# manuelruder/fast-artistic-videos

Hardware: AMD Instinct MI355X
Metric: stylized frames/sec @1280x720, per-frame hot path (mask + warp + assembly + net + deprocess + PNG encode on the GPU) with inputs resident in HBM; file->PNG rate of the product CLI (BASELINE.json's end-to-end) in `end_to_end_fps` / `e2e`, PSNR vs CPU ref in `parity` (higher is better)
Workload: dtype f32

## Files before the change

fast-artistic-videos_amd/csrc/fav_internal.h:

```cpp
#pragma once
#include <hip/hip_runtime.h>
#include <cstdarg>
#include <cstdint>
#include <cstdio>
#include <exception>
#include <new>
#include <string>
#include <vector>

#include "../../include/fav.h"

#include <cstdlib>
inline const char* diag_env(const char* name)
{
#ifdef FAV_DIAG
    return getenv(name);
#else
    (void)name;
    return nullptr;
#endif
}

namespace fav {

void set_error(const char* fmt, ...);
int hip_fail(hipError_t e, const char* what);

#define FAV_HIP(expr)                                              \
    do {                                                           \
        hipError_t e__ = (expr);                                   \
        if (e__ != hipSuccess) return ::fav::hip_fail(e__, #expr); \
    } while (0)
#define FAV_LAUNCH_CHECK(name)                                            \
    do {                                                                  \
        hipError_t e__ = hipGetLastError();                               \
        if (e__ != hipSuccess) return ::fav::hip_fail(e__, "launch " name); \
    } while (0)
#define FAV_REQUIRE(cond, ...)                 \
    do {                                       \
        if (!(cond)) {                         \
            ::fav::set_error(__VA_ARGS__);     \
            return FAV_EINVAL;                 \
        }                                      \
    } while (0)

#define FAV_ABI_TRY try {
#define FAV_ABI_CATCH(where_)                                                                                            \
    } catch (const std::bad_alloc&) {                                                                                   \
        ::fav::set_error(where_ ": out of memory while parsing (damaged size field?)"); return FAV_EFORMAT;                \
    } catch (const std::exception& e__) {                                                                               \
        ::fav::set_error(where_ ": %s", e__.what()); return FAV_EFORMAT;                                                  \
    } catch (...) {                                                                                                     \
        ::fav::set_error(where_ ": unexpected exception"); return FAV_EFORMAT;                                            \
    }

int ensure_device();

struct TraceRange {
    explicit TraceRange(const char* name);
    ~TraceRange();
    static bool enabled();
    bool on;
};

enum LayerType { L_PAD, L_CONV, L_IN, L_RELU, L_RES, L_UP, L_TANH, L_MUL, L_IDENTITY, L_BN };

struct Layer {
    LayerType type = L_IDENTITY;
    int pl = 0, pr = 0, pt = 0, pb = 0, pad_mode = 0;
    int cin = 0, cout = 0, k = 0, stride = 1, pad = 0;
    int transposed = 0, adj = 0;
    std::vector<float> w, b;
    std::vector<float> gamma, beta, mean, var;
    float eps = 1e-5f;
    int scale = 1;
    float mul = 1.f;
    int shave = 0;
    std::vector<Layer> block;
};

int t7_parse_model(const char* path, std::vector<Layer>& out);
int blob_pack(const std::vector<Layer>& layers, std::vector<uint8_t>& blob);
int blob_unpack(const void* blob, size_t bytes, std::vector<Layer>& out);
std::string describe_layers(const std::vector<Layer>& layers, int indent = 0);

struct Affine {
    const float* scale1 = nullptr; const float* shift1 = nullptr; int relu1 = 0;
    const float* scale2 = nullptr; const float* shift2 = nullptr; int relu2 = 0;
    int stages = 0;
    const long long* acc1 = nullptr; long long* acc1_zero = nullptr;
    const float* gamma1 = nullptr; const float* beta1 = nullptr; float eps1 = 0.f; int count1 = 0;
};
constexpr int STAT_COPIES = 8;
inline size_t stat_acc_words(int C) { return (size_t)STAT_COPIES * C * 4; }
constexpr long long STAT_NONFINITE = 1ll << 53;
__host__ __device__ inline bool stat_acc_poisoned(long long hi_sum, long long hi_squares)
{
    return hi_sum >= STAT_NONFINITE / 2 || hi_sum <= -(STAT_NONFINITE / 2) || hi_squares >= STAT_NONFINITE / 2 || hi_squares <= -(STAT_NONFINITE / 2);
}

struct ConvLaunch {
    const float* in = nullptr;
    int IH = 0, IW = 0;
    int IWp = 0;
    int ups = 0;
    int stuff = 0;
    int CIN = 0;
    Affine pre;
    const float* wgt = nullptr;
    const unsigned short* wgt16 = nullptr;
    const float* bias = nullptr;
    int COUT = 0, COUTp = 0;
    int KH = 0, KW = 0, stride = 1, pad = 0;
    int Kpad = 0;
    int OH = 0, OW = 0;
    float* out = nullptr;
    float* partials = nullptr;
    int final_mode = 0;
    float tanh_mul = 1.f;
    float* out_planar = nullptr;
    float* out_raw_nchw = nullptr;
    float* sk_ws = nullptr; unsigned* sk_flags = nullptr; unsigned sk_epoch = 0;
    unsigned* sk_err = nullptr;
    int reserve_cus = 0;
    int no_sk = 0;
    const float* join_skip = nullptr; float* join_out = nullptr; int OWp = 0;
    long long* stat_acc = nullptr;
    float* ks_ws = nullptr; int* ks_cnt = nullptr;
};
inline size_t conv3_wino4_ksplit_bytes() { return (size_t)256 * 2 * 256 * 128 * sizeof(float); }
size_t conv_streamk_workspace_bytes();
int conv_streamk_grid();
constexpr int CONV_BM = 128;
inline int conv_mblocks(int OH, int OW) { return (OH * OW + CONV_BM - 1) / CONV_BM; }
int launch_conv(const ConvLaunch& p, hipStream_t st);
bool conv_c8_eligible(int cin_pitch, int coutp, int k, int stride, int stages, int ups);
int conv_c8_tiles(int OH, int OW);
int launch_conv_c8(const ConvLaunch& p, int* counts, hipStream_t st);
bool conv_c8d_eligible(int cin_pitch, int cin_real, int coutp, int k, int stride, int stages, int ups);
void conv_c8d_pack(const float* w, int cin, int cout, std::vector<float>& out);
int launch_conv_c8d(const ConvLaunch& p, int cin_real, const float* wc8d, int* counts, hipStream_t st);
bool conv3_halo_eligible(int cin_pitch, int coutp, int k, int stride);
int conv3_halo_tiles(int OH, int OW, bool edge_b);
int launch_conv3_halo(const ConvLaunch& p, int* counts, hipStream_t st);
bool conv3s2_eligible(int cin_pitch, int coutp, int k, int stride, int stages, int ups);
int conv3s2_tiles(int OH, int OW);
int launch_conv3s2(const ConvLaunch& p, int* counts, hipStream_t st);
bool conv_fold_eligible(int cin_pitch, int cout, int k, int stride);
bool conv_fold_launchable(int cin_pitch, int k, int pad, int ups, int IH, int IW);
int launch_conv_fold(const ConvLaunch& p, const float* wfold, hipStream_t st);
int conv_first_tiles(int OH, int OW);
int launch_conv_first(const ConvLaunch& p, int cin_real, const float* wpk, int* counts, hipStream_t st);
bool conv_first2d_eligible(int cin_pitch, int cin_real, int coutp, int k, int stride, int stages, int ups);
int conv_first2d_tiles(int OH, int OW);
int launch_conv_first2d(const ConvLaunch& p, int cin_real, const float* wpk, int* counts, hipStream_t st);
bool conv3_wino_eligible(int cin_pitch, int cout, int coutp, int k, int stride, int pad, int stages, int ups);
int conv3_wino_tiles(int OH, int OW);
int launch_conv3_wino(const ConvLaunch& p, const float* wpk, int* counts, hipStream_t st);
bool conv3_wino4_eligible(int cin_pitch, int cout, int coutp, int k, int stride, int pad, int stages, int ups);
int conv3_wino4_tiles(int OH, int OW);
int launch_conv3_wino4(const ConvLaunch& p, const float* wpk, int* counts, hipStream_t st);
bool conv3_up2_eligible(int cin_pitch, int cout, int coutp, int k, int stride, int pad, int stages, int ups);
int conv3_up2_tiles(int OH, int OW);
int launch_conv3_up2(const ConvLaunch& p, const float* wpk, int* counts, hipStream_t st);
bool conv3s2w_eligible(int cin_pitch, int cout, int coutp, int k, int stride, int pad, int stages, int ups);
int conv3s2w_tiles(int OH, int OW, int coutp);
int launch_conv3s2w(const ConvLaunch& p, const float* wpk, int* counts, hipStream_t st);
enum ConvKernel { CK_GENERIC, CK_FOLD, CK_C8, CK_C8D, CK_FIRST1D, CK_FIRST2D, CK_S2W, CK_UP2, CK_WINO, CK_WINO4, CK_HALO3, CK_S2HALO };
constexpr int CONV_KERNELS = CK_S2HALO + 1;
int launch_in_finalize(const float* partials, const int* counts, int mblocks, int M, int block_pixels, int C, int Cpitch,
                       const float* gamma, const float* beta, float eps,
                       float* scale, float* shift, hipStream_t st);
int launch_stats(const float* x, int M, int C, const Affine& t, float* partials, hipStream_t st);
int launch_pad_nhwc(const float* in, int Hp, int Wp, int in_pitch, int C, int ups, float* out, int pl, int pr, int pt, int pb, int mode, hipStream_t st);
int launch_res_add(const float* y, const float* scale, const float* shift,
                   const float* skip, int SH, int SW, int shave, const Affine& skip_t,
                   int C, float* z, float* partials, int* counts, hipStream_t st, int skip_pitch = 0, const Affine* branch_acc = nullptr);
inline int res_add_stat_blocks(int OH, int OW) { return OH * ((OW + 127) / 128); }
int launch_nchw_to_nhwc_pad(const float* in, int C, int H, int W, int pad, int Cp, float* out, hipStream_t st);
int launch_nhwc_to_nchw(const float* in, int M, int C, const Affine& t, float* out, hipStream_t st);

#ifdef __HIPCC__
__device__ __forceinline__ float fill_uniform(unsigned seed, unsigned index, unsigned c, unsigned y, unsigned x)
{
    unsigned k = seed * 0x9E3779B1u + index * 0x85EBCA77u + c * 0xC2B2AE3Du + y * 0x27D4EB2Fu + x * 0x165667B1u;
    k ^= k >> 15; k *= 0x2C1B3C6Du;
    k ^= k >> 12; k *= 0x297A2D39u;
    k ^= k >> 15;
    return (float)(k >> 8) * (1.0f / 16777216.0f);
}
#endif

int launch_warp(const float* img, const float* flow, float* out, int B, int C, int H, int W, int Ho, int Wo,
                int border, hipStream_t st);
int launch_min_filter_f32(const float* cert, float* out, int H, int W, int r, hipStream_t st);
int launch_assemble(const float* frame, const float* warped, const float* cert, float* in7, int H, int W,
                    hipStream_t st);
int launch_cert_prepare(const uint8_t* mask, const float* backward_flo, int invert, int fix_occ, int border,
                        int r, float* cert_tmp, float* cert, int H, int W, hipStream_t st);
int launch_prep_input(const uint8_t* frame_hwc, const float* prev_rgb, int Hs, int Ws, const float* backward_flo,
                      const float* cert, int border, int H, int W, int pad, float* in8, hipStream_t st,
                      int fill_random = 0, unsigned seed = 0, unsigned index = 0, int* q0_out = nullptr);
int launch_quantize_rgb8(const float* rgb_planar, uint8_t* out_hwc, int H, int W, hipStream_t st);
int launch_scale_prep(const uint8_t* frame_hwc, int H, int W, int Hs, int Ws, int pad, float* in8, hipStream_t st,
                      int fill_random = 0, unsigned seed = 0, unsigned index = 0);
int launch_scale_planar(const float* src, float* dst, int C, int Hs, int Ws, int Hd, int Wd, hipStream_t st);
constexpr int PNG_NSYM = 277;
constexpr int PNG_NTABLES = 12;
constexpr int PNG_HDR_WORDS = 40;
struct PngTable {
    uint32_t sym[PNG_NSYM];
    uint32_t hdr[PNG_HDR_WORDS];
    uint32_t hdr_bits, btype, dist_len, dist_code;
};
const std::vector<PngTable>& png_tables();
size_t png_capacity(int W, int H);
size_t png_workspace_bytes(int W, int H);
uint32_t png_crc32_combine_host(uint32_t crc_a, uint32_t crc_b, uint32_t len_b);
int launch_png_encode(const uint8_t* rgb_hwc, const float* rgb_planar, int W, int H, void* png_out, size_t capacity, uint32_t* png_bytes,
                      void* workspace, size_t ws_bytes, hipStream_t st);
int launch_check_cert(const float* backward_flo, const float* forward_flo, const float* structure, const float* avg, uint8_t* mask_out,
                      int invert, int fix_occ, int border, int r, float* cert, int H, int W, hipStream_t st);
int launch_check_prep(const uint8_t* frame_hwc, const float* prev_rgb, int Hs, int Ws, const float* backward_flo, const float* forward_flo,
                      const float* structure, const float* avg, uint8_t* mask_out, float* cert, int invert, int fix_occ, int border, int r,
                      int H, int W, int pad, float* in8, hipStream_t st, int fill_random, unsigned seed, unsigned index);
int launch_store_flag(uint32_t* flag_host, uint32_t value, hipStream_t st);
int launch_unpad_input(const float* in8, int H, int W, int pad, float* in7, hipStream_t st);
int launch_temporal_loss(const float* prev_rgb, const float* cur_rgb, const float* backward_flo, const uint8_t* cert_u8, int border,
                         int H, int W, double* partial256, hipStream_t st);

size_t structure_workspace_bytes(int W, int H);
int launch_structure(const uint8_t* rgb_hwc, int W, int H, void* ws, size_t ws_bytes,
                     const float** structure_out, const float** avg_out, hipStream_t st, int pack_cus = 0, const int* q0_main = nullptr);
int launch_sequential_sum(const float* x, size_t n, float* sum_out, hipStream_t st);
int launch_consistency(const float* f1_flo, const float* f2_flo, const float* structure, const float* avg,
                       uint8_t* out, int W, int H, hipStream_t st);

int launch_vr_rotate(const float* src, float* dst, int H, int W, int mode, hipStream_t st);
int launch_vr_accum(float* acc, const float* w, const float* div, size_t n, int first, hipStream_t st);
int launch_vr_cert(const uint8_t* cert_u8, const float* m0, const float* m1, const float* m2, const float* m3, float* out, size_t n,
                   hipStream_t st);
int launch_vr_prior(const float* lfw, const float* border, const float* grad, const float* cert, const float* m, const float* m2,
                    float* out, size_t n, hipStream_t st);
int launch_vr_blend(const float* seg, const float* borders, const float* g, const float* anti, float* out, size_t n, hipStream_t st);
int launch_vr_median(const float* src, float* dst, int H, int W, int r, hipStream_t st);
int launch_vr_strip(const float* face, int FH, int FW, int cy, int cx, int CH, int CW, int mode, float* strip, int SH, int SW,
                    int x0, hipStream_t st);
int launch_vr_prep(const uint8_t* frame_hwc, const float* prior, const float* cert, int fill_random, unsigned seed, unsigned index,
                   int H, int W, int pad, float* in8, hipStream_t st);
int launch_vr_flo_to_lua(const float* flo_uv, float* lua_dydx, size_t n, hipStream_t st);

}

struct fav_net;
namespace fav {
int net_device(const fav_net* n);
int net_pad(const fav_net* n);
int net_in_channels(const fav_net* n);
void net_out_size(const fav_net* n, int H, int W, int* Ho, int* Wo);
int net_forward_padded(fav_net* n, const float* in8, int H, int W, float* out_planar, hipStream_t st);
void net_forget_stream(const fav_net* n, hipStream_t st);
void net_reserve_cus(fav_net* n, int cus);
}
```

fast-artistic-videos_amd/csrc/kernels_elem.hip:

```cpp
#include <algorithm>

#include "fav_internal.h"
#include "conv_device.h"

namespace fav {

namespace {

__global__ __launch_bounds__(256) void in_finalize_kernel(const float2* partials, const int* counts, int mblocks, int M, int bp,
                                                          int Cpitch, const float* gamma, const float* beta,
                                                          float eps, float* scale, float* shift)
{
    __shared__ double sh[8];
    const int c = blockIdx.x, t = threadIdx.x;
    double s1 = 0, s2 = 0;
    float gq = 1.f, bq = 0.f;
    if (t == 0) { gq = gamma ? gamma[c] : 1.f; bq = beta ? beta[c] : 0.f; }
    for (int b0 = t; b0 < mblocks; b0 += 1024) {
        float2 pr[4]; int nb[4];
#pragma unroll
        for (int k = 0; k < 4; ++k) {
            const int b = b0 + 256 * k, bc = min(b, mblocks - 1);
            pr[k] = partials[(size_t)bc * Cpitch + c];
            nb[k] = b < mblocks ? (counts ? counts[bc] : min(bp, M - bc * bp)) : 0;
        }
#pragma unroll
        for (int k = 0; k < 4; ++k) {
            const double n = (double)nb[k], mu = (double)pr[k].x;
            s1 += n * mu;
            s2 += (nb[k] ? (double)pr[k].y : 0.0) + n * mu * mu;
        }
    }
    for (int o = 32; o > 0; o >>= 1) { s1 += __shfl_xor(s1, o); s2 += __shfl_xor(s2, o); }
    if ((t & 63) == 0) { sh[2 * (t >> 6)] = s1; sh[2 * (t >> 6) + 1] = s2; }
    __syncthreads();
    if (t == 0) {
        const double a = ((sh[0] + sh[2]) + sh[4]) + sh[6], q = ((sh[1] + sh[3]) + sh[5]) + sh[7];
        const double mean = a / (double)M;
        double var = q / (double)M - mean * mean;
        var = var > 0.0 ? var : 0.0;
        const double g = (double)gq, bt = (double)bq;
        const double sc = g / sqrt(var + (double)eps);
        scale[c] = (float)sc;
        shift[c] = (float)(bt - mean * sc);
    }
}

__device__ __forceinline__ float4 apply_affine_g(float4 v, const Affine& a, int c)
{
    if (a.stages >= 1) {
        v = affine4(v, a.scale1 + c, a.shift1 + c, a.relu1);
        if (a.stages >= 2) v = affine4(v, a.scale2 + c, a.shift2 + c, a.relu2);
    }
    return v;
}

template <int NPT>
__global__ __launch_bounds__(256) void stats_kernel(const float* x, int M, int C, const Affine a, float2* partials)
{
    __shared__ float red[1024];
    __shared__ float mean_s[1024];
    const int t = threadIdx.x;
    const int groups = C >> 2;
    const int nl = 256 / groups;
    const int g = t % groups, pl = t / groups;
    const int m0 = blockIdx.x * 128;
    const int cnt = min(128, M - m0);
    const bool active = pl < nl;
    float4 s = make_float4(0, 0, 0, 0);
    float4 keep[NPT > 0 ? NPT : 1];
    if (NPT > 0) {
#pragma unroll
        for (int i = 0; i < NPT; ++i) {
            const int pix = pl + i * nl;
            float4 v = make_float4(0, 0, 0, 0);
            if (pix < cnt) { v = *reinterpret_cast<const float4*>(x + (size_t)(m0 + pix) * C + 4 * g); v = apply_affine_g(v, a, 4 * g); }
            keep[i] = v;
        }
#pragma unroll
        for (int i = 0; i < NPT; ++i) { s.x += keep[i].x; s.y += keep[i].y; s.z += keep[i].z; s.w += keep[i].w; }
    } else if (active)
        for (int pix = pl; pix < cnt; pix += nl) {
            float4 v = *reinterpret_cast<const float4*>(x + (size_t)(m0 + pix) * C + 4 * g);
            v = apply_affine_g(v, a, 4 * g);
            s.x += v.x; s.y += v.y; s.z += v.z; s.w += v.w;
        }
    if (active) *reinterpret_cast<float4*>(red + pl * C + 4 * g) = s;
    __syncthreads();
    for (int c = t; c < C; c += 256) {
        float r = 0;
        for (int i = 0; i < nl; ++i) r += red[i * C + c];
        mean_s[c] = r / (float)cnt;
    }
    __syncthreads();
    float4 q = make_float4(0, 0, 0, 0);
    if (active) {
        const float4 mu = *reinterpret_cast<const float4*>(mean_s + 4 * g);
        if (NPT > 0) {
#pragma unroll
            for (int i = 0; i < NPT; ++i) {
                const float4 v = keep[i];
                const float dx = v.x - mu.x, dy = v.y - mu.y, dz = v.z - mu.z, dw = v.w - mu.w;
                if (pl + i * nl < cnt) { q.x = fmaf(dx, dx, q.x); q.y = fmaf(dy, dy, q.y); q.z = fmaf(dz, dz, q.z); q.w = fmaf(dw, dw, q.w); }
            }
        } else
            for (int pix = pl; pix < cnt; pix += nl) {
                float4 v = *reinterpret_cast<const float4*>(x + (size_t)(m0 + pix) * C + 4 * g);
                v = apply_affine_g(v, a, 4 * g);
                const float dx = v.x - mu.x, dy = v.y - mu.y, dz = v.z - mu.z, dw = v.w - mu.w;
                q.x = fmaf(dx, dx, q.x); q.y = fmaf(dy, dy, q.y); q.z = fmaf(dz, dz, q.z); q.w = fmaf(dw, dw, q.w);
            }
        *reinterpret_cast<float4*>(red + pl * C + 4 * g) = q;
    }
    __syncthreads();
    for (int c = t; c < C; c += 256) {
        float r = 0;
        for (int i = 0; i < nl; ++i) r += red[i * C + c];
        partials[(size_t)blockIdx.x * C + c] = make_float2(mean_s[c], r);
    }
}

template <bool ACC>
__global__ __launch_bounds__(256) void res_add_kernel(const float* y, const float* scale, const float* shift,
                                                      const float* skip, int SW, int shave, const Affine sa,
                                                      int OH, int OW, int C, float* z, const Affine br)
{
    __shared__ float ss[ACC ? 2048 : 4];
    if (ACC) {
        for (int i = threadIdx.x; i < C; i += 256) {
            long long w0 = 0, w1 = 0, w2 = 0, w3 = 0;
#pragma unroll
            for (int cp = 0; cp < STAT_COPIES; ++cp) {
                const longlong2* a = reinterpret_cast<const longlong2*>(br.acc1 + ((size_t)cp * C + i) * 4);
                const longlong2 lo = a[0], hi = a[1];
                w0 += lo.x; w1 += lo.y; w2 += hi.x; w3 += hi.y;
            }
            const double s1 = ((double)w1 * 4294967296.0 + (double)w0) * (1.0 / 1099511627776.0);
            const double s2 = ((double)w3 * 4294967296.0 + (double)w2) * (1.0 / 1099511627776.0);
            const double mean = s1 / (double)br.count1;
            double var = s2 / (double)br.count1 - mean * mean;
            var = var > 0.0 ? var : 0.0;
            const double sc = stat_acc_poisoned(w1, w3) ? (double)NAN : (double)br.gamma1[i] / sqrt(var + (double)br.eps1);
            ss[i] = (float)sc; ss[C + i] = (float)((double)br.beta1[i] - mean * sc);
            if (blockIdx.x == 0) {
#pragma unroll
                for (int cp = 0; cp < STAT_COPIES; ++cp) {
                    longlong2* zz = reinterpret_cast<longlong2*>(br.acc1_zero + ((size_t)cp * C + i) * 4);
                    zz[0] = longlong2{0, 0}; zz[1] = longlong2{0, 0};
                }
            }
        }
        __syncthreads();
        scale = ss; shift = ss + C;
    }
    const int groups = C >> 2;
    const size_t total = (size_t)OH * OW * groups;
    for (size_t idx = (size_t)blockIdx.x * 256 + threadIdx.x; idx < total; idx += (size_t)gridDim.x * 256) {
        const int g = (int)(idx % groups);
        const size_t pix = idx / groups;
        const int oy = (int)(pix / OW), ox = (int)(pix - (size_t)oy * OW);
        float4 v = *reinterpret_cast<const float4*>(y + pix * C + 4 * g);
        v = affine4(v, scale + 4 * g, shift + 4 * g, 0);
        float4 k = *reinterpret_cast<const float4*>(skip + ((size_t)(oy + shave) * SW + ox + shave) * C + 4 * g);
        k = apply_affine_g(k, sa, 4 * g);
        v.x += k.x; v.y += k.y; v.z += k.z; v.w += k.w;
        *reinterpret_cast<float4*>(z + pix * C + 4 * g) = v;
    }
}

template <int NPT>
__global__ __launch_bounds__(256) void res_add_stats_kernel(const float* y, const float* scale, const float* shift,
                                                            const float* skip, int SW, int shave, const Affine sa,
                                                            int OW, int C, float* z, float2* partials, int* counts)
{
    __shared__ float red[1024];
    __shared__ float mean_s[1024];
    const int t = threadIdx.x;
    const int groups = C >> 2, nl = 256 / groups;
    const int g = t % groups, pl = t / groups;
    const int segs = (OW + 127) / 128;
    const int oy = blockIdx.x / segs, x0 = (blockIdx.x - oy * segs) * 128;
    const int cnt = min(128, OW - x0);
    const bool active = pl < nl;
    const float* yr = y + ((size_t)oy * OW + x0) * C + 4 * g;
    const float* kr = skip + ((size_t)(oy + shave) * SW + x0 + shave) * C + 4 * g;
    float* zr = z + ((size_t)oy * OW + x0) * C + 4 * g;
    float4 sm = make_float4(0, 0, 0, 0);
    float4 keep[NPT > 0 ? NPT : 1];
    if (NPT > 0) {
        float4 kk[NPT > 0 ? NPT : 1];
#pragma unroll
        for (int i = 0; i < NPT; ++i) {
            const int px = pl + i * nl;
            keep[i] = make_float4(0, 0, 0, 0); kk[i] = make_float4(0, 0, 0, 0);
            if (px < cnt) { keep[i] = *reinterpret_cast<const float4*>(yr + (size_t)px * C); kk[i] = *reinterpret_cast<const float4*>(kr + (size_t)px * C); }
        }
#pragma unroll
        for (int i = 0; i < NPT; ++i) {
            const int px = pl + i * nl;
            float4 v = affine4(keep[i], scale + 4 * g, shift + 4 * g, 0);
            const float4 k = apply_affine_g(kk[i], sa, 4 * g);
            v.x += k.x; v.y += k.y; v.z += k.z; v.w += k.w;
            if (px < cnt) { *reinterpret_cast<float4*>(zr + (size_t)px * C) = v; sm.x += v.x; sm.y += v.y; sm.z += v.z; sm.w += v.w; }
            keep[i] = v;
        }
    } else if (active)
        for (int px = pl; px < cnt; px += nl) {
            float4 v = *reinterpret_cast<const float4*>(yr + (size_t)px * C);
            v = affine4(v, scale + 4 * g, shift + 4 * g, 0);
            float4 k = *reinterpret_cast<const float4*>(kr + (size_t)px * C);
            k = apply_affine_g(k, sa, 4 * g);
            v.x += k.x; v.y += k.y; v.z += k.z; v.w += k.w;
            *reinterpret_cast<float4*>(zr + (size_t)px * C) = v;
            sm.x += v.x; sm.y += v.y; sm.z += v.z; sm.w += v.w;
        }
    if (active) *reinterpret_cast<float4*>(red + pl * C + 4 * g) = sm;
    __syncthreads();
    for (int c = t; c < C; c += 256) {
        float r = 0;
        for (int i = 0; i < nl; ++i) r += red[i * C + c];
        mean_s[c] = r / (float)cnt;
    }
    __syncthreads();
    float4 q = make_float4(0, 0, 0, 0);
    if (active) {
        const float4 mu = *reinterpret_cast<const float4*>(mean_s + 4 * g);
        if (NPT > 0) {
#pragma unroll
            for (int i = 0; i < NPT; ++i) {
                const float4 v = keep[i];
                const float dx = v.x - mu.x, dy = v.y - mu.y, dz = v.z - mu.z, dw = v.w - mu.w;
                if (pl + i * nl < cnt) { q.x = fmaf(dx, dx, q.x); q.y = fmaf(dy, dy, q.y); q.z = fmaf(dz, dz, q.z); q.w = fmaf(dw, dw, q.w); }
            }
        } else
        for (int px = pl; px < cnt; px += nl) {
            const float4 v = *reinterpret_cast<const float4*>(zr + (size_t)px * C);
            const float dx = v.x - mu.x, dy = v.y - mu.y, dz = v.z - mu.z, dw = v.w - mu.w;
            q.x = fmaf(dx, dx, q.x); q.y = fmaf(dy, dy, q.y); q.z = fmaf(dz, dz, q.z); q.w = fmaf(dw, dw, q.w);
        }
        *reinterpret_cast<float4*>(red + pl * C + 4 * g) = q;
    }
    __syncthreads();
    for (int c = t; c < C; c += 256) {
        float r = 0;
        for (int i = 0; i < nl; ++i) r += red[i * C + c];
        partials[(size_t)blockIdx.x * C + c] = make_float2(mean_s[c], r);
    }
    if (t == 0) counts[blockIdx.x] = cnt;
}

__device__ __forceinline__ int reflect(int i, int n)
{
    if (i < 0) i = -i;
    if (i >= n) i = 2 * (n - 1) - i;
    return i;
}

__global__ __launch_bounds__(256) void nchw_to_nhwc_pad_kernel(const float* in, int C, int H, int W, int pad, int Cp,
                                                               float* out)
{
    const int Hp = H + 2 * pad, Wp = W + 2 * pad;
    const size_t total = (size_t)Hp * Wp * Cp;
    for (size_t idx = (size_t)blockIdx.x * 256 + threadIdx.x; idx < total; idx += (size_t)gridDim.x * 256) {
        const int c = (int)(idx % Cp);
        const size_t pix = idx / Cp;
        const int y = (int)(pix / Wp), x = (int)(pix - (size_t)y * Wp);
        float v = 0.f;
        if (c < C) v = in[((size_t)c * H + reflect(y - pad, H)) * W + reflect(x - pad, W)];
        out[idx] = v;
    }
}

__global__ __launch_bounds__(256) void nhwc_to_nchw_kernel(const float* in, int M, int C, const Affine a, float* out)
{
    const size_t total = (size_t)M * C;
    for (size_t idx = (size_t)blockIdx.x * 256 + threadIdx.x; idx < total; idx += (size_t)gridDim.x * 256) {
        const int c = (int)(idx / M);
        const size_t m = idx - (size_t)c * M;
        float v = in[m * C + c];
        if (a.stages >= 1) {
            v = fmaf(v, a.scale1[c], a.shift1[c]); if (a.relu1) v = fmaxf(v, 0.f);
            if (a.stages >= 2) { v = fmaf(v, a.scale2[c], a.shift2[c]); if (a.relu2) v = fmaxf(v, 0.f); }
        }
        out[idx] = v;
    }
}

inline int grid_for(size_t total) { size_t b = (total + 255) / 256; return (int)(b > 8192 ? 8192 : (b ? b : 1)); }

}

int launch_in_finalize(const float* partials, const int* counts, int mblocks, int M, int block_pixels, int C, int Cpitch,
                       const float* gamma, const float* beta, float eps, float* scale, float* shift, hipStream_t st)
{
    hipLaunchKernelGGL(in_finalize_kernel, dim3(C), dim3(256), 0, st, reinterpret_cast<const float2*>(partials), counts,
                       mblocks, M, block_pixels, Cpitch, gamma, beta, eps, scale, shift);
    FAV_LAUNCH_CHECK("in_finalize_kernel");
    return FAV_OK;
}

int launch_stats(const float* x, int M, int C, const Affine& t, float* partials, hipStream_t st)
{
    FAV_REQUIRE(C % 4 == 0 && C <= 1024 && 256 % (C / 4) == 0, "stats: unsupported channel count %d", C);
    const dim3 grid((M + 127) / 128);
    float2* pp = reinterpret_cast<float2*>(partials);
    if (C == 64) hipLaunchKernelGGL(stats_kernel<8>, grid, dim3(256), 0, st, x, M, C, t, pp);
    else if (C == 128) hipLaunchKernelGGL(stats_kernel<16>, grid, dim3(256), 0, st, x, M, C, t, pp);
    else hipLaunchKernelGGL(stats_kernel<0>, grid, dim3(256), 0, st, x, M, C, t, pp);
    FAV_LAUNCH_CHECK("stats_kernel");
    return FAV_OK;
}

int launch_res_add(const float* y, const float* scale, const float* shift, const float* skip, int SH, int SW,
                   int shave, const Affine& skip_t, int C, float* z, float* partials, int* counts, hipStream_t st, int skip_pitch, const Affine* branch_acc)
{
    const int OH = SH - 2 * shave, OW = SW - 2 * shave;
    if (skip_pitch > 0) SW = skip_pitch;
    FAV_REQUIRE(C % 4 == 0 && C <= 1024 && 256 % (C / 4) == 0 && OH > 0 && OW > 0, "res_add: bad shape (C=%d)", C);
    FAV_REQUIRE(!(partials && branch_acc && branch_acc->acc1), "res_add: the statistics-taking join does not take an accumulator-form InstanceNorm");
    if (partials) {
        const dim3 grid(res_add_stat_blocks(OH, OW));
        float2* pp = reinterpret_cast<float2*>(partials);
        if (C == 128) hipLaunchKernelGGL(res_add_stats_kernel<16>, grid, dim3(256), 0, st, y, scale, shift, skip, SW, shave, skip_t, OW, C, z, pp, counts);
        else if (C == 64) hipLaunchKernelGGL(res_add_stats_kernel<8>, grid, dim3(256), 0, st, y, scale, shift, skip, SW, shave, skip_t, OW, C, z, pp, counts);
        else hipLaunchKernelGGL(res_add_stats_kernel<0>, grid, dim3(256), 0, st, y, scale, shift, skip, SW, shave, skip_t, OW, C, z, pp, counts);
    }
    else if (branch_acc != nullptr && branch_acc->acc1 != nullptr)
        hipLaunchKernelGGL(res_add_kernel<true>, dim3(std::min(1024, grid_for((size_t)OH * OW * (C / 4)))), dim3(256), 0, st, y, scale, shift, skip, SW, shave, skip_t,
                           OH, OW, C, z, *branch_acc);
    else
        hipLaunchKernelGGL(res_add_kernel<false>, dim3(grid_for((size_t)OH * OW * (C / 4))), dim3(256), 0, st, y, scale, shift, skip, SW, shave, skip_t,
                           OH, OW, C, z, Affine());
    FAV_LAUNCH_CHECK("res_add_kernel");
    return FAV_OK;
}

int launch_nchw_to_nhwc_pad(const float* in, int C, int H, int W, int pad, int Cp, float* out, hipStream_t st)
{
    FAV_REQUIRE(pad < H && pad < W, "reflection pad %d must be smaller than the image (%dx%d)", pad, W, H);
    hipLaunchKernelGGL(nchw_to_nhwc_pad_kernel, dim3(grid_for((size_t)(H + 2 * pad) * (W + 2 * pad) * Cp)), dim3(256), 0,
                       st, in, C, H, W, pad, Cp, out);
    FAV_LAUNCH_CHECK("nchw_to_nhwc_pad_kernel");
    return FAV_OK;
}

int launch_nhwc_to_nchw(const float* in, int M, int C, const Affine& t, float* out, hipStream_t st)
{
    hipLaunchKernelGGL(nhwc_to_nchw_kernel, dim3(grid_for((size_t)M * C)), dim3(256), 0, st, in, M, C, t, out);
    FAV_LAUNCH_CHECK("nhwc_to_nchw_kernel");
    return FAV_OK;
}

}
```

fast-artistic-videos_amd/csrc/kernels_wino4.hip:

```cpp
#include <algorithm>
#include <cstdlib>
#include <type_traits>
#include <vector>

#include "fav_internal.h"
#include "wino4_pack.h"

namespace fav {

typedef float v4f __attribute__((ext_vector_type(4)));
typedef int v4i __attribute__((ext_vector_type(4)));

namespace {

constexpr int MAX_DEVICES = 64;
constexpr int W4_MEET_MAX = 256;
constexpr int W4_SHARES = 252;
inline int cur_dev() { int d = 0; (void)hipGetDevice(&d); return (d >= 0 && d < MAX_DEVICES) ? d : 0; }

constexpr int W4_VPOS = 256;
constexpr int W4_VBUF = 36 * W4_VPOS;
constexpr int W4_LLINE = 18 * 4;
constexpr int W4_LTY = 113 * 4;
constexpr int W4_LKQ = 464 * 4;
constexpr int W4_LBUF = 4 * W4_LKQ;
constexpr int W4_RBUF = 6 * 288 * 4;
constexpr int W4_SMEM = 2 * W4_VBUF + W4_LBUF + W4_RBUF;
static_assert((W4_LTY / 4) % 16 == 1 && (W4_LKQ / 4) % 16 == 0 && W4_LTY >= 6 * W4_LLINE && W4_LKQ >= 4 * W4_LTY, "pitches of L");

struct Wino4Args {
    const float* in; const float* wpk; const float* bias; const float* scale1; const float* shift1;
    float* out; float2* partials; int* counts;
    const float* skip; float* zout;
    int OWp;
    int IH, IW, IWp, CIN, OH, OW, units_x, units_y, relu1;
    int stream, shares; float* ks_ws; int* ks_cnt;
    long long* dbg;
    long long* stat_acc; const long long* acc1; long long* acc1_zero; const float* gamma1; const float* beta1; float eps1; int count1;
    int COUT, groups;
};

__device__ __forceinline__ void w4_store16_wt(void* ptr, v4f v)
{
    asm volatile("global_store_dwordx4 %0, %1, off sc1" ::"v"(ptr), "v"(v) : "memory");
}

typedef float v2f __attribute__((ext_vector_type(2)));
__device__ __forceinline__ v2f w4_fma(float a, v2f b, v2f c) { return __builtin_elementwise_fma(v2f{a, a}, b, c); }
__device__ __forceinline__ void w4_bt2(const v2f d[6], v2f v[6])
{
    const v2f e1 = w4_fma(-2.25f, d[2], d[4]), o1 = w4_fma(-1.6875f, d[1], 0.75f * d[3]);
    const v2f e2 = w4_fma(-0.5625f, d[2], d[4]), o2 = w4_fma(-0.84375f, d[1], 1.5f * d[3]);
    v[0] = w4_fma(1.265625f, d[0], w4_fma(-2.8125f, d[2], d[4]));
    v[1] = e1 + o1; v[2] = e1 - o1; v[3] = e2 + o2; v[4] = e2 - o2;
    v[5] = w4_fma(1.265625f, d[1], w4_fma(-2.8125f, d[3], d[5]));
}
__device__ __forceinline__ void w4_bt(const v4f d[6], v4f v[6])
{
    v2f dl[6], dh[6], vl[6], vh[6];
#pragma unroll
    for (int i = 0; i < 6; ++i) { dl[i] = d[i].xy; dh[i] = d[i].zw; }
    w4_bt2(dl, vl); w4_bt2(dh, vh);
#pragma unroll
    for (int i = 0; i < 6; ++i) v[i] = v4f{vl[i].x, vl[i].y, vh[i].x, vh[i].y};
}
__device__ __forceinline__ void w4_at(const v2f m[6], v2f y[4])
{
    const v2f s1 = m[1] + m[2], d1 = m[1] - m[2], s2 = m[3] + m[4], d2 = m[3] - m[4];
    y[0] = (m[0] + s1) + s2;
    y[1] = w4_fma(1.5f, d2, 0.75f * d1);
    y[2] = w4_fma(2.25f, s2, 0.5625f * s1);
    y[3] = w4_fma(3.375f, d2, w4_fma(0.421875f, d1, m[5]));
}

template <int MODE, int VAR = 0, bool WIDE = false>
__global__ __launch_bounds__(512) __attribute__((amdgpu_waves_per_eu(2, 2))) void conv3_wino4_kernel(const Wino4Args p)
{
    constexpr bool AFF = MODE != 0, JOIN = MODE == 2;
    constexpr bool PAIR = (VAR & 8) == 0 && MODE != 2;
    constexpr int NT = 512;
    extern __shared__ __attribute__((aligned(16))) float smem[];
    float* const Vs = smem;
    float* const Ls = smem + 2 * W4_VBUF;
    float* const Rs = Ls + W4_LBUF;
    float* const Ss = Rs + W4_RBUF;
    float* const aff = Ss + ((MODE == 2 || PAIR) ? W4_RBUF : 0);
    typedef __attribute__((address_space(3))) void* lds_ptr_t;

    const int t = threadIdx.x, lane = t & 63;
    const int wave = __builtin_amdgcn_readfirstlane(t >> 6);
    const int CIN = p.CIN, nslices = CIN >> 4;

    int dbi = 0;
#define DBG_T() { if (p.dbg && t == 0 && dbi < 21) p.dbg[blockIdx.x * 24 + dbi++] = wall_clock64(); }
    DBG_T();
    int lb;
    {
        const int nwg = gridDim.x, q = nwg >> 3, r = nwg & 7, xcd = blockIdx.x & 7, idx = blockIdx.x >> 3;
        lb = (xcd < r ? xcd * (q + 1) : r * (q + 1) + (xcd - r) * q) + idx;
    }
    if (MODE == 1 && p.acc1 != nullptr) {
        for (int i = t; i < CIN; i += NT) {
            long long w0 = 0, w1 = 0, w2 = 0, w3 = 0;
#pragma unroll
            for (int cp = 0; cp < STAT_COPIES; ++cp) {
                const longlong2* a = reinterpret_cast<const longlong2*>(p.acc1 + ((size_t)cp * CIN + i) * 4);
                const longlong2 lo = a[0], hi = a[1];
                w0 += lo.x; w1 += lo.y; w2 += hi.x; w3 += hi.y;
            }
            const double s1 = ((double)w1 * 4294967296.0 + (double)w0) * (1.0 / 1099511627776.0);
            const double s2 = ((double)w3 * 4294967296.0 + (double)w2) * (1.0 / 1099511627776.0);
            const double mean = s1 / (double)p.count1;
            double var = s2 / (double)p.count1 - mean * mean;
            var = var > 0.0 ? var : 0.0;
            const double sc = stat_acc_poisoned(w1, w3) ? (double)NAN : (double)p.gamma1[i] / sqrt(var + (double)p.eps1);
            aff[i] = (float)sc; aff[CIN + i] = (float)((double)p.beta1[i] - mean * sc);
            if (blockIdx.x == 0) {
#pragma unroll
                for (int cp = 0; cp < STAT_COPIES; ++cp) {
                    longlong2* z = reinterpret_cast<longlong2*>(p.acc1_zero + ((size_t)cp * CIN + i) * 4);
                    z[0] = longlong2{0, 0}; z[1] = longlong2{0, 0};
                }
            }
        }
    } else if (AFF) for (int i = t; i < CIN; i += NT) { aff[i] = p.scale1[i]; aff[CIN + i] = p.shift1[i]; }
    const float lo1 = (MODE == 1 && p.relu1) ? 0.f : -INFINITY;

    const bool has1 = t < 288;
    const int cq = (t >> 3) & 3;
    const int pix1 = min((t >> 5) * 8 + (t & 7), 71), ty1 = (pix1 * 3641) >> 16, x1 = pix1 - ty1 * 18;
    float* const l1 = Ls + cq * W4_LKQ + ty1 * W4_LTY + x1 * 4;
    const float* const affr = aff + cq * 4;
    const bool has2 = wave >= 2;
    const int i2 = max(wave - 2, 0);
    const int m2 = lane & 15, kq2 = lane >> 4;
    const float* const l2 = Ls + kq2 * W4_LKQ + (m2 >> 2) * W4_LTY + 4 * (m2 & 3) * 4 + i2 * W4_LLINE;
    float* const v2 = Vs + lane * 4 + 6 * i2 * W4_VPOS;
    const float* const aA = Vs + lane * 4;
    const int wlo = lane * 16, wso = wave * 1024;

    v4f fb[6];
    bool ring_primed = false;
    int ring_grp = 0;
    const int upix = p.units_x * p.units_y;
    if (AFF) __syncthreads();
    auto work = [&](const int ug, const int s0, const int s1, const int meet, const int part) {
        const int nsl = s1 - s0;
        const bool whole = meet < 0;
        if (s0 != 0) ring_primed = false;
        int u = ug, grp = 0;
        if (WIDE) {
            if (p.stream) { grp = ug / upix; u = ug - grp * upix; } else { u = ug / p.groups; grp = ug - u * p.groups; }
            if (grp != ring_grp) { ring_primed = false; ring_grp = grp; }
        }
        const int wgb = (p.CIN >> 4) * 36 * 8192;
        const __amdgpu_buffer_rsrc_t wrs = __builtin_amdgcn_make_buffer_rsrc(const_cast<float*>(p.wpk) + (WIDE ? (size_t)grp * (wgb >> 2) : 0), 0, wgb, 0x00020000);
        const __amdgpu_buffer_rsrc_t irs = __builtin_amdgcn_make_buffer_rsrc(const_cast<float*>(p.in), 0, p.IH * p.IWp * p.CIN * 4, 0x00020000);
        const __amdgpu_buffer_rsrc_t srs = __builtin_amdgcn_make_buffer_rsrc(const_cast<float*>(JOIN ? p.skip : p.in), 0, p.IH * p.IWp * p.CIN * 4, 0x00020000);
        const __amdgpu_buffer_rsrc_t zrs = __builtin_amdgcn_make_buffer_rsrc(JOIN ? p.zout : const_cast<float*>(p.in), 0, p.IH * p.IWp * p.CIN * 4, 0x00020000);
        const int uy = u / p.units_x, ux = u - uy * p.units_x;
        const int oy0 = uy * 16, ox0 = ux * 16;
        DBG_T();
        const int ho0 = ((min(oy0 + 4 * ty1, p.IH - 1) * p.IWp + min(ox0 + x1, p.IW - 1)) * CIN + cq * 4) * 4;
        const int hrmax = max(p.IH - 1 - (oy0 + 4 * ty1), 0);
        const int hrow = p.IWp * CIN * 4;
#define ho_(a_) (ho0 + min((a_), hrmax) * hrow)
        const int dpix = min(t >> 2, 71), dty = (dpix * 3641) >> 16, dx = dpix - dty * 18;
        const int hd0 = ((min(oy0 + 4 * dty, p.IH - 1) * p.IWp + min(ox0 + dx, p.IW - 1)) * CIN + (t & 3) * 4) * 4;
        const int hdmax = max(p.IH - 1 - (oy0 + 4 * dty), 0);
#define hd_(a_) (hd0 + min((a_), hdmax) * hrow)
        int zm = 0;
        const bool lastx = ux == p.units_x - 1, lasty = uy == p.units_y - 1;
        if (JOIN) {
            const bool cv = ox0 + x1 < p.IW && (x1 < 16 || lastx);
#pragma unroll
            for (int a = 0; a < 6; ++a) zm |= (cv && oy0 + 4 * ty1 + a < p.IH && (a < 4 || (ty1 == 3 && lasty)) ? 1 : 0) << a;
        }

        v4f sc, sh;
        float* const land = Rs + wave * 256;
        const float* const rread = Rs + (pix1 * 4 + cq) * 4;
        constexpr int RROW = 288 * 4;
        constexpr int SKO = W4_RBUF;
#define W4_LOAD_RAW(q_, slice_)                                                                     \
        { _Pragma("unroll") for (int a = 0; a < 6; ++a) q_[a] = __builtin_bit_cast(v4f, __builtin_amdgcn_raw_buffer_load_b128(irs, ho_(a), (slice_) * 64, 0)); }
#define W4_LOAD_SKIP(x_, slice_)                                                                    \
        { if (JOIN) { _Pragma("unroll") for (int a = 0; a < 6; ++a) x_[a] = __builtin_bit_cast(v4f, __builtin_amdgcn_raw_buffer_load_b128(srs, ho_(a), (slice_) * 64, 0)); } }
#define W4_REQ_RAW(slice_)                                                                          \
        { asm volatile("" ::: "memory");       \
          if (JOIN) { _Pragma("unroll") for (int a = 0; a < 6; ++a)      \
              __builtin_amdgcn_raw_ptr_buffer_load_lds(srs, (lds_ptr_t)(land + SKO + a * RROW), 16, hd_(a), (slice_) * 64, 0, 0); } \
          _Pragma("unroll") for (int a = 0; a < 6; ++a)                                             \
              __builtin_amdgcn_raw_ptr_buffer_load_lds(irs, (lds_ptr_t)(land + a * RROW), 16, hd_(a), (slice_) * 64, 0, 0); }
#define W4_TAKE_RAW(q_)                                                                             \
        { _Pragma("unroll") for (int a = 0; a < 6; ++a) q_[a] = *reinterpret_cast<const v4f*>(rread + a * RROW); }
        constexpr int RROW2 = 576 * 4;
        const float* const rread2 = Rs + (pix1 * 8 + cq) * 4;
        float* const land2 = Rs + wave * 512;
#define W4_REQ_PAIR(a_)                                                                             \
        { asm volatile("" ::: "memory");                                                            \
          int ln_ = lane; asm volatile("" : "+v"(ln_));                                             \
          _Pragma("unroll") for (int j = 0; j < 2; ++j) { if (j == 0 || wave < 4) {                 \
              const int dp_ = 16 * wave + 8 * j + (ln_ >> 3), dy_ = (dp_ * 3641) >> 16, dx_ = dp_ - 18 * dy_;                     \
              const int b_ = ((min(oy0 + 4 * dy_, p.IH - 1) * p.IWp + min(ox0 + dx_, p.IW - 1)) * CIN + (ln_ & 7) * 4) * 4;       \
              const int mx_ = max(p.IH - 1 - (oy0 + 4 * dy_), 0);                                   \
              _Pragma("unroll") for (int a = 0; a < 6; ++a)                                         \
                  __builtin_amdgcn_raw_ptr_buffer_load_lds(irs, (lds_ptr_t)(land2 + j * 256 + a * RROW2), 16, b_ + min(a, mx_) * hrow, (a_) * 64, 0, 0); } } }
#define W4_TAKE_PAIR(q_, slice_)                                                                    \
        { const float* const rr_ = rread2 + ((slice_) & 1) * 16;                                     \
          _Pragma("unroll") for (int a = 0; a < 6; ++a) q_[a] = *reinterpret_cast<const v4f*>(rr_ + a * RROW2); }
#define W4_SKIP_LDS(a_) (*reinterpret_cast<const v4f*>(rread + SKO + (a_) * RROW))
#define W4_AFF(slice_)                                                                              \
        { if (AFF) { sc = *reinterpret_cast<const v4f*>(affr + (slice_) * 16); sh = *reinterpret_cast<const v4f*>(affr + CIN + (slice_) * 16); } }
#define W4_PEND(q_, xs_, slice_)                                                                    \
        { _Pragma("unroll") for (int a = 0; a < 6; ++a) {                                           \
            if (MODE == 1) { const v2f fl_ = __builtin_elementwise_fma(q_[a].xy, sc.xy, sh.xy), fh_ = __builtin_elementwise_fma(q_[a].zw, sc.zw, sh.zw); \
                             q_[a].x = fmaxf(fl_.x, lo1); q_[a].y = fmaxf(fl_.y, lo1); q_[a].z = fmaxf(fh_.x, lo1); q_[a].w = fmaxf(fh_.y, lo1); } \
            if (JOIN) { const v4f x1_ = xs_(a);                                                     \
                        q_[a].x = fmaf(q_[a].x, sc.x, sh.x) + x1_.x; q_[a].y = fmaf(q_[a].y, sc.y, sh.y) + x1_.y;                \
                        q_[a].z = fmaf(q_[a].z, sc.z, sh.z) + x1_.z; q_[a].w = fmaf(q_[a].w, sc.w, sh.w) + x1_.w;                \
                        if (!(VAR & 16) && (a < 4 || lasty)) __builtin_amdgcn_raw_buffer_store_b128(__builtin_bit_cast(v4i, q_[a]), zrs, (zm & (1 << a)) ? ho_(a) : (int)0xFFFFFFF0, (slice_) * 64, 0); } } }
#define W4_COMMIT1(q_)                                                                              \
        { v4f l_[6]; w4_bt(q_, l_);                                                                 \
          _Pragma("unroll") for (int i = 0; i < 6; ++i) *reinterpret_cast<v4f*>(l1 + i * W4_LLINE) = l_[i]; }
#define W4_S2_READ(c_)                                                                              \
        { _Pragma("unroll") for (int k = 0; k < 6; ++k) c_[k] = *reinterpret_cast<const v4f*>(l2 + k * 4); }
#define W4_S2_DONE(c_, nb_)                                                                         \
        { v4f o_[6]; w4_bt(c_, o_);                                                                 \
          _Pragma("unroll") for (int j = 0; j < 6; ++j) *reinterpret_cast<v4f*>(v2 + (nb_) * W4_VBUF + j * W4_VPOS) = o_[j]; }

        v4f fa[4];
#define W4_READ_A(slot_, par_, pos_) { fa[slot_] = *reinterpret_cast<const v4f*>(aA + (par_) * W4_VBUF + (pos_) * W4_VPOS); }
#define W4_LOAD_B(slot_, sl_, pos_)                                                                 \
        { fb[slot_] = __builtin_bit_cast(v4f, __builtin_amdgcn_raw_buffer_load_b128(wrs, wlo, wso + ((sl_) * 36 + (pos_)) * 8192, 0)); }

        {
            v4f qa[6], xa[6];
            if (has1) { W4_LOAD_SKIP(xa, s0); W4_LOAD_RAW(qa, s0); }
            if (!ring_primed) {
#pragma unroll
                for (int q = 0; q < 4; ++q) { W4_LOAD_B(q, s0, q); }
                ring_primed = true;
            }
            if (has1) {
                W4_AFF(s0);
#define W4_SKIP_REG(a_) xa[a_]
                W4_PEND(qa, W4_SKIP_REG, s0); W4_COMMIT1(qa);
#undef W4_SKIP_REG
                if (!PAIR) W4_REQ_RAW(min(s0 + 1, s1 - 1));
            }
            if (PAIR && wave < 5) W4_REQ_PAIR((s0 + 1) & ~1);
            __syncthreads();
            if (has2) { v4f c2[6]; W4_S2_READ(c2); W4_S2_DONE(c2, 0); }
        }
        v4f acc[36];
#pragma unroll
        for (int q = 0; q < 36; ++q) acc[q] = v4f{0.f, 0.f, 0.f, 0.f};
        __syncthreads();
        W4_READ_A(0, 0, 0); W4_READ_A(1, 0, 1);
        DBG_T();
        const long long ck0 = p.dbg ? clock64() : 0, wk0 = p.dbg ? wall_clock64() : 0;

#define W4_FENCE() __builtin_amdgcn_sched_barrier(0)
#define W4_POSITIONS(from_, to_)                                                                    \
        { _Pragma("unroll") for (int pos = (from_); pos < (to_); pos += 2) {                       \
            if (pos + 2 < 36) { W4_READ_A((pos + 2) % 4, par, pos + 2); W4_READ_A((pos + 3) % 4, par, pos + 3); }    \
            if (!(VAR & 1)) {                                                                       \
            if (pos + 4 < 36) { W4_LOAD_B((pos + 4) % 6, s, pos + 4); } else { W4_LOAD_B((pos + 4) % 6, sw, pos + 4 - 36); } \
            if (pos + 5 < 36) { W4_LOAD_B((pos + 5) % 6, s, pos + 5); } else { W4_LOAD_B((pos + 5) % 6, sw, pos + 5 - 36); } } \
            W4_FENCE();                                                                             \
            _Pragma("unroll") for (int j = 0; j < 4; ++j) {                                         \
                acc[pos] = __builtin_amdgcn_mfma_f32_16x16x4f32(fa[pos % 4][j], fb[pos % 6][j], acc[pos], 0, 0, 0); \
                acc[pos + 1] = __builtin_amdgcn_mfma_f32_16x16x4f32(fa[(pos + 1) % 4][j], fb[(pos + 1) % 6][j], acc[pos + 1], 0, 0, 0); \
            }                                                                                       \
            W4_FENCE(); } }
        for (int sl = 0; sl < nsl; ++sl) {
            const int s = s0 + sl, par = sl & 1;
            const int sn = min(s + 1, s1 - 1);
            const int sw = s + 1 < s1 ? s + 1 : 0;
            const int sn2 = min(s + 2, s1 - 1);
            W4_POSITIONS(0, 6);
            if (sl == 0) {
                if (PAIR ? wave < 5 : has1) asm volatile("s_waitcnt vmcnt(6)" ::: "memory");
                __syncthreads();
            }
            if (PAIR) {
                if (has1) { v4f qa[6]; W4_TAKE_PAIR(qa, sn); W4_AFF(sn); W4_PEND(qa, W4_SKIP_LDS, sn); W4_COMMIT1(qa); }
                if (wave < 5 && !(s & 1) && s + 2 < s1) W4_REQ_PAIR(s + 2);
            } else
            if (!(VAR & 2) && has1) {
                v4f qa[6];
                W4_TAKE_RAW(qa);
                W4_AFF(sn); W4_PEND(qa, W4_SKIP_LDS, sn); W4_COMMIT1(qa);
                W4_REQ_RAW(sn2);
            }
            W4_POSITIONS(6, 12);
            if (!(VAR & 4)) __syncthreads();
            W4_POSITIONS(12, 14);
            if (!(VAR & 2) && has2) { v4f c2[6]; W4_S2_READ(c2); W4_S2_DONE(c2, par ^ 1); }
            W4_POSITIONS(14, 36);
            if (PAIR ? wave < 5 : has1) asm volatile("s_waitcnt vmcnt(6)" ::: "memory");
            if (!(VAR & 4)) __syncthreads();
            W4_READ_A(0, par ^ 1, 0); W4_READ_A(1, par ^ 1, 1);
        }
#undef W4_POSITIONS
#undef W4_FENCE
        DBG_T();
        if (p.dbg && t == 0) { p.dbg[blockIdx.x * 24 + 21] += clock64() - ck0; p.dbg[blockIdx.x * 24 + 22] += wall_clock64() - wk0; }
        DBG_T();
#undef ho_
#undef hd_
#undef W4_LOAD_RAW
#undef W4_REQ_RAW
#undef W4_TAKE_RAW
#undef W4_REQ_PAIR
#undef W4_TAKE_PAIR
#undef W4_SKIP_LDS
#undef W4_S2_READ
#undef W4_S2_DONE
#undef W4_LOAD_SKIP
#undef W4_AFF
#undef W4_PEND
#undef W4_COMMIT1
#undef W4_READ_A
#undef W4_LOAD_B

        const int cn = lane & 15, g = lane >> 4;
        const int nrows = max(0, min(16, p.OH - oy0)), ncols = max(0, min(16, p.OW - ox0));
        const int nv = nrows * ncols;
        const int cpb = WIDE ? p.COUT * 4 : 512;
        const __amdgpu_buffer_rsrc_t ors = __builtin_amdgcn_make_buffer_rsrc(p.out, 0, p.OH * p.OWp * cpb, 0x00020000);
        const bool inside = nv == 256;
        const int oyb = oy0 + 4 * g;
        const int cb = (WIDE ? grp * 128 : 0) + wave * 16 + cn;
        float y[4][4][4];
        {
            const float bv = whole ? p.bias[cb] : 0.f;
            const v2f bv2 = v2f{bv, bv};
#pragma unroll
            for (int r = 0; r < 4; r += 2) {
                v2f Q[4][6];
#pragma unroll
                for (int j = 0; j < 6; ++j) {
                    const v2f mcol[6] = {r ? acc[j].zw : acc[j].xy, r ? acc[6 + j].zw : acc[6 + j].xy, r ? acc[12 + j].zw : acc[12 + j].xy,
                                         r ? acc[18 + j].zw : acc[18 + j].xy, r ? acc[24 + j].zw : acc[24 + j].xy, r ? acc[30 + j].zw : acc[30 + j].xy};
                    v2f o[4]; w4_at(mcol, o);
                    Q[0][j] = o[0]; Q[1][j] = o[1]; Q[2][j] = o[2]; Q[3][j] = o[3];
                }
#pragma unroll
                for (int a = 0; a < 4; ++a) {
                    v2f o[4]; w4_at(Q[a], o);
#pragma unroll
                    for (int b = 0; b < 4; ++b) { const v2f ob = o[b] + bv2; y[a][b][r] = ob.x; y[a][b][r + 1] = ob.y; }
                }
            }
        }
        if (!whole) {
            float* const mine = p.ks_ws + ((size_t)meet * 2 + part) * 32768 + (wave * 64 + lane) * 4;
            const float* const other = p.ks_ws + ((size_t)meet * 2 + (part ^ 1)) * 32768 + (wave * 64 + lane) * 4;
            int* const flag = reinterpret_cast<int*>(aff + 2 * CIN);
            if (t == 0) *flag = __hip_atomic_load(p.ks_cnt + meet, __ATOMIC_RELAXED, __HIP_MEMORY_SCOPE_AGENT);
            __syncthreads();
            bool second = *flag == 1;
            __syncthreads();
            if (!second) {
#pragma unroll
                for (int a = 0; a < 4; ++a)
#pragma unroll
                    for (int b = 0; b < 4; ++b)
                        w4_store16_wt(mine + (a * 4 + b) * 2048, v4f{y[a][b][0], y[a][b][1], y[a][b][2], y[a][b][3]});
                asm volatile("s_waitcnt vmcnt(0)" ::: "memory");
                __syncthreads();
                if (t == 0) *flag = __hip_atomic_fetch_add(p.ks_cnt + meet, 1, __ATOMIC_RELAXED, __HIP_MEMORY_SCOPE_AGENT);
                __syncthreads();
                second = *flag == 1;
                __syncthreads();
                if (!second) { DBG_T(); return; }
            }
            __builtin_amdgcn_fence(__ATOMIC_ACQUIRE, "agent");
            if (t == 0) __hip_atomic_store(p.ks_cnt + meet, 0, __ATOMIC_RELAXED, __HIP_MEMORY_SCOPE_AGENT);
            const float bv = p.bias[cb];
#pragma unroll
            for (int a = 0; a < 4; ++a)
#pragma unroll
                for (int b = 0; b < 4; ++b) {
                    const v4f o = *reinterpret_cast<const v4f*>(other + (a * 4 + b) * 2048);
                    y[a][b][0] = (y[a][b][0] + o.x) + bv; y[a][b][1] = (y[a][b][1] + o.y) + bv;
                    y[a][b][2] = (y[a][b][2] + o.z) + bv; y[a][b][3] = (y[a][b][3] + o.w) + bv;
                }
        }
        float sm = 0.f, mu = 0.f, m2 = 0.f;
        if (inside) {
#pragma unroll
            for (int a = 0; a < 4; ++a) {
                const int ro = ((oyb + a) * p.OWp + ox0) * cpb + cb * 4;
#pragma unroll
                for (int r = 0; r < 4; ++r)
#pragma unroll
                    for (int b = 0; b < 4; ++b) {
                        __builtin_amdgcn_raw_buffer_store_b32(__builtin_bit_cast(int, y[a][b][r]), ors, ro + r * 4 * cpb + b * cpb, 0, 0);
                        sm += y[a][b][r];
                    }
            }
            if (p.partials != nullptr) {
                sm += __shfl_xor(sm, 16); sm += __shfl_xor(sm, 32);
                mu = sm * (1.f / 256.f);
#pragma unroll
                for (int a = 0; a < 4; ++a)
#pragma unroll
                    for (int r = 0; r < 4; ++r)
#pragma unroll
                        for (int b = 0; b < 4; ++b) { const float d = y[a][b][r] - mu; m2 = fmaf(d, d, m2); }
            }
        } else {
#pragma unroll
            for (int a = 0; a < 4; ++a) {
                const bool rv = oyb + a < p.OH;
                const int ro = rv ? ((oyb + a) * p.OWp + ox0) * cpb + cb * 4 : (int)0xFFFF0000;
#pragma unroll
                for (int c = 0; c < 16; ++c) {
                    if (c < ncols) {
                        const float v = y[a][c & 3][c >> 2];
                        __builtin_amdgcn_raw_buffer_store_b32(__builtin_bit_cast(int, v), ors, ro + c * cpb, 0, 0);
                        sm += rv ? v : 0.f;
                    }
                }
            }
            if (p.partials != nullptr) {
                sm += __shfl_xor(sm, 16); sm += __shfl_xor(sm, 32);
                mu = nv ? sm / (float)nv : 0.f;
#pragma unroll
                for (int a = 0; a < 4; ++a) {
                    const bool rv = oyb + a < p.OH;
#pragma unroll
                    for (int c = 0; c < 16; ++c) {
                        if (c < ncols) {
                            const float d = y[a][c & 3][c >> 2] - mu;
                            m2 = rv ? fmaf(d, d, m2) : m2;
                        }
                    }
                }
            }
        }
        if (p.partials != nullptr) {
            m2 += __shfl_xor(m2, 16); m2 += __shfl_xor(m2, 32);
            if (p.stat_acc != nullptr) {
                const double nd = (double)nv, mud = (double)mu;
                const double v = (g & 2) ? (double)m2 + nd * mud * mud : nd * mud;
                const double tt = v * 1099511627776.0;
                const double hi = floor(tt * (1.0 / 4294967296.0));
                const bool fin = fabs(tt) < 9.0e18;
                const long long word = !fin ? ((g & 1) ? STAT_NONFINITE : 0ll) : (g & 1) ? (long long)hi : (long long)(tt - hi * 4294967296.0);
                long long* const dst = p.stat_acc + ((size_t)(blockIdx.x & (STAT_COPIES - 1)) * (WIDE ? p.COUT : 128) + cb) * 4 + g;
                __hip_atomic_fetch_add(dst, word, __ATOMIC_RELAXED, __HIP_MEMORY_SCOPE_AGENT);
            } else if (g == 0) p.partials[(size_t)u * (WIDE ? p.COUT : 128) + cb] = make_float2(mu, m2);
        }
        if (p.partials != nullptr && p.stat_acc == nullptr && t == 0 && grp == 0) p.counts[u] = nv;
        DBG_T();
    };
    const int units = WIDE ? upix * p.groups : upix;
    if (!p.stream) {
        for (int u = lb; u < units; u += gridDim.x) work(u, 0, nslices, -1, 0);
    } else {
        const long long tot = (long long)units * nslices;
        for (int sh = lb; sh < p.shares; sh += gridDim.x) {
            int g = (int)(tot * sh / p.shares);
            const int g1 = (int)(tot * (sh + 1) / p.shares);
            while (g < g1) {
                const int u = g / nslices, s0 = g - u * nslices, s1 = min(nslices, s0 + (g1 - g));
                const bool whole = s0 == 0 && s1 == nslices;
                work(u, s0, s1, whole ? -1 : (s0 == 0 ? sh : sh - 1), s0 == 0 ? 0 : 1);
                g += s1 - s0;
            }
        }
    }
    if (p.dbg && t == 0) p.dbg[blockIdx.x * 24 + 23] = dbi;
#undef DBG_T
}

void wino4_debug_report(const long long* hbuf, int grid, int mode)
{
    long long t0 = hbuf[0];
    for (int b = 0; b < grid; ++b) t0 = std::min(t0, hbuf[b * 24]);
    double sum[4] = {0, 0, 0, 0}, tend = 0, ck = 0, wk = 0; int items = 0;
    for (int b = 0; b < grid; ++b) {
        const long long* r = &hbuf[b * 24]; const int n = (int)r[23];
        for (int i = 1; i + 4 < n + 1 && i + 4 <= 20; i += 5) {
            for (int q = 0; q < 4; ++q) sum[q] += (r[i + q + 1] - r[i + q]) * 0.01;
            ++items; tend = std::max(tend, (r[i + 4] - t0) * 0.01);
        }
        ck += r[21]; wk += r[22];
    }
    fprintf(stderr, "WINO4DBG mode=%d grid=%d units=%d  K loop: %.3f GHz;  per unit: prologue %.2f  loop %.2f  epilogue %.2f us;  last block ends at %.2f us\n",
            mode, grid, items, wk ? ck / (wk * 10.0) : 0.0, items ? sum[0] / items : 0.0, items ? sum[1] / items : 0.0, items ? sum[3] / items : 0.0, tend);
}

template <int MODE, bool WIDE>
int launch_wino4_t(const Wino4Args& a0, int reserve_cus, hipStream_t st)
{
#ifdef FAV_DIAG
    static const int var = diag_env("FAV_W4_VAR") ? atoi(diag_env("FAV_W4_VAR")) : 0;
    const auto kern = (!WIDE && MODE == 1 && var == 1) ? conv3_wino4_kernel<1, 1> : (!WIDE && MODE == 1 && var == 2) ? conv3_wino4_kernel<1, 2> : (!WIDE && MODE == 1 && var == 3) ? conv3_wino4_kernel<1, 3> :
                      (!WIDE && MODE == 1 && var == 7) ? conv3_wino4_kernel<1, 7> : (!WIDE && MODE == 1 && var == 6) ? conv3_wino4_kernel<1, 6> :
                      (!WIDE && MODE == 2 && var == 16) ? conv3_wino4_kernel<2, 16> :
                      (MODE != 2 && var == 8) ? conv3_wino4_kernel<MODE, MODE != 2 ? 8 : 0, WIDE> : conv3_wino4_kernel<MODE, 0, WIDE>;
    const bool pair = MODE != 2 && !(var & 8);
#else
    const auto kern = conv3_wino4_kernel<MODE, 0, WIDE>;
    const bool pair = MODE != 2;
#endif
    const size_t lds = (size_t)(W4_SMEM + ((MODE == 2 || pair) ? W4_RBUF : 0) + 2 * a0.CIN + 4) * sizeof(float);
    const int dv = cur_dev();
    static int cus[MAX_DEVICES] = {};
    if (!cus[dv]) {
        FAV_HIP(hipFuncSetAttribute(reinterpret_cast<const void*>(kern), hipFuncAttributeMaxDynamicSharedMemorySize, 160 * 1024));
        int occ = 0; int prop_cus = 0;
        FAV_HIP(hipDeviceGetAttribute(&prop_cus, hipDeviceAttributeMultiprocessorCount, dv));
        FAV_HIP(hipOccupancyMaxActiveBlocksPerMultiprocessor(&occ, reinterpret_cast<const void*>(kern), 512, lds));
        if (occ < 1) { set_error("winograd F(4x4) conv: kernel does not fit on a CU"); return FAV_EHIP; }
        cus[dv] = prop_cus;
    }
    const int units = a0.units_x * a0.units_y * (WIDE ? a0.groups : 1);
    int grid = std::min(units, std::max(1, cus[dv] - reserve_cus));
    Wino4Args a = a0; a.dbg = nullptr;
    static const bool no_stream = diag_env("FAV_W4_NO_STREAM") != nullptr;
    static const int grid_cap = diag_env("FAV_W4_GRID") ? atoi(diag_env("FAV_W4_GRID")) : 0;
    if (grid_cap > 0) grid = std::min(grid, std::max(1, grid_cap));
    const int shares = grid_cap > 0 ? std::max(1, std::min(W4_SHARES, grid_cap)) : W4_SHARES;
    const int rounds = (units + shares - 1) / shares, rem = units - (rounds - 1) * shares;
    a.stream = (rounds >= 2 && rem * 5 <= shares * 3 && shares <= W4_MEET_MAX && a0.ks_ws && a0.ks_cnt && !no_stream) ? 1 : 0;
    a.shares = shares;
    if (a.stream) grid = std::min(grid, shares);
    static int dbg_n = diag_env("FAV_WINO_DBG") ? atoi(diag_env("FAV_WINO_DBG")) : 0;
    static long long* dbuf = nullptr;
    const bool dbg = dbg_n > 0 && --dbg_n == 0;
    if (dbg) { FAV_HIP(hipMalloc(reinterpret_cast<void**>(&dbuf), 512 * 24 * 8)); FAV_HIP(hipMemsetAsync(dbuf, 0, 512 * 24 * 8, st)); a.dbg = dbuf; }
    hipLaunchKernelGGL(kern, dim3(grid), dim3(512), lds, st, a);
    FAV_LAUNCH_CHECK("conv3_wino4_kernel");
    if (dbg) {
        std::vector<long long> hb((size_t)512 * 24);
        FAV_HIP(hipStreamSynchronize(st)); FAV_HIP(hipMemcpy(hb.data(), dbuf, hb.size() * 8, hipMemcpyDeviceToHost));
        wino4_debug_report(hb.data(), grid, MODE);
    }
    return FAV_OK;
}

}

bool conv3_wino4_eligible(int cin_pitch, int cout, int coutp, int k, int stride, int pad, int stages, int ups)
{
    return k == 3 && stride == 1 && pad == 0 && ups == 0 && stages <= 1 && cin_pitch % 16 == 0 && cin_pitch >= 16 && cin_pitch <= 512 &&
           cout == coutp && cout % 128 == 0 && cout >= 128 && cout <= 1024;
}
int conv3_wino4_tiles(int OH, int OW) { return ((OH + 15) / 16) * ((OW + 15) / 16); }

int launch_conv3_wino4(const ConvLaunch& c, const float* wpk, int* counts, hipStream_t st)
{
    FAV_REQUIRE(conv3_wino4_eligible(c.CIN, c.COUT, c.COUTp, c.KH, c.stride, c.pad, c.pre.stages, c.ups) && c.KH == c.KW && !c.final_mode && !c.stuff && wpk,
                "winograd F(4x4) conv: not eligible");
    FAV_REQUIRE((long long)(c.IH + 1) * c.IWp * c.CIN < (1ll << 29), "winograd F(4x4) conv: tensor too large for 32-bit byte offsets");
    FAV_REQUIRE(c.OH == c.IH - 2 && c.OW == c.IW - 2, "winograd F(4x4) conv: bad geometry");
    FAV_REQUIRE((long long)(c.OH + 1) * (c.OWp > 0 ? c.OWp : c.OW) * c.COUT < (1ll << 29), "winograd F(4x4) conv: output too large for 32-bit byte offsets");
    Wino4Args a;
    a.in = c.in; a.wpk = wpk; a.bias = c.bias; a.scale1 = c.pre.scale1; a.shift1 = c.pre.shift1; a.relu1 = c.pre.relu1;
    a.out = c.out; a.partials = reinterpret_cast<float2*>(c.partials); a.counts = counts;
    a.IH = c.IH; a.IW = c.IW; a.IWp = c.IWp; a.CIN = c.CIN; a.OH = c.OH; a.OW = c.OW;
    a.units_x = (c.OW + 15) / 16; a.units_y = (c.OH + 15) / 16;
    a.dbg = nullptr;
    a.skip = c.join_skip; a.zout = c.join_out; a.OWp = c.OWp > 0 ? c.OWp : c.OW;
    a.ks_ws = c.ks_ws; a.ks_cnt = c.ks_cnt; a.stream = 0; a.shares = 1;
    a.COUT = c.COUT; a.groups = c.COUT / 128;
    a.stat_acc = c.stat_acc; a.acc1 = c.pre.acc1; a.acc1_zero = c.pre.acc1_zero; a.gamma1 = c.pre.gamma1; a.beta1 = c.pre.beta1; a.eps1 = c.pre.eps1; a.count1 = c.pre.count1;
    if (c.stat_acc != nullptr && a.partials == nullptr) a.partials = reinterpret_cast<float2*>(c.stat_acc);
    FAV_REQUIRE(c.pre.acc1 == nullptr || (c.join_skip == nullptr && c.pre.stages == 1 && c.pre.count1 > 0), "winograd F(4x4) conv: accumulator-form InstanceNorm on an unsupported input");
    if (c.join_skip != nullptr) {
        FAV_REQUIRE(c.join_out != nullptr && c.pre.stages == 1 && c.pre.relu1 == 0, "winograd F(4x4) conv: a pending residual join needs its output tensor and exactly one pending normalisation");
        FAV_REQUIRE(a.groups == 1, "winograd F(4x4) conv: a pending residual join is formed by 128-filter layers only");
        return launch_wino4_t<2, false>(a, c.reserve_cus, st);
    }
    if (a.groups > 1) return c.pre.stages >= 1 ? launch_wino4_t<1, true>(a, c.reserve_cus, st) : launch_wino4_t<0, true>(a, c.reserve_cus, st);
    return c.pre.stages >= 1 ? launch_wino4_t<1, false>(a, c.reserve_cus, st) : launch_wino4_t<0, false>(a, c.reserve_cus, st);
}

}
```

fast-artistic-videos_amd/csrc/net.cpp:

```cpp
#include <algorithm>
#include <cmath>
#include <cstdlib>
#include <cstring>
#include <functional>
#include <memory>

#include <mutex>

#include "fav_internal.h"
#include "wino_pack.h"
#include "wino4_pack.h"
#include "up2_pack.h"
#include "s2_pack.h"
#include "first_pack.h"
#include "first2d_pack.h"
#include "fold_pack.h"

using namespace fav;

namespace {

struct DevBuf { void* p = nullptr; size_t bytes = 0; };
struct DevConvW {
    float* wgt = nullptr; float* bias = nullptr; unsigned short* wgt16 = nullptr;
    float* packed[CONV_KERNELS] = {};
    int cinp = 0, coutp = 0, kpad = 0;
};
struct DevIN { float* gamma = nullptr; float* beta = nullptr; float* scale = nullptr; float* shift = nullptr;
               long long* acc = nullptr; size_t acc_bytes = 0; };

struct Act {
    float* data = nullptr;
    int Hp = 0, Wp = 0;
    int C = 0;
    int ups = 0;
    Affine pre;
    float* partials = nullptr;
    int mblocks = 0, ppitch = 0;
    int* counts = nullptr;
    int pitch = 0;
    const float* join_skip = nullptr; float* join_out = nullptr;
    long long* acc = nullptr; long long* acc_other = nullptr;
    int H() const { return Hp << ups; }
    int W() const { return Wp << ups; }
    int P() const { return pitch ? pitch : Wp; }
};

int dev_upload(const std::vector<float>& h, size_t pad_to, float** out)
{
    const size_t n = std::max(pad_to, h.size());
    std::vector<float> tmp(n, 0.f);
    std::copy(h.begin(), h.end(), tmp.begin());
    FAV_HIP(hipMalloc(reinterpret_cast<void**>(out), (n ? n : 1) * sizeof(float)));
    if (n) FAV_HIP(hipMemcpy(*out, tmp.data(), n * sizeof(float), hipMemcpyHostToDevice));
    return FAV_OK;
}

void repack_weights(const Layer& L, int cinp, int coutp, int kpad, std::vector<float>& out)
{
    out.assign((size_t)coutp * kpad, 0.f);
    const int taps = L.k * L.k;
    for (int co = 0; co < L.cout; ++co)
        for (int ci = 0; ci < L.cin; ++ci)
            for (int ky = 0; ky < L.k; ++ky)
                for (int kx = 0; kx < L.k; ++kx) {
                    const int tap = ky * L.k + kx;
                    const size_t k = cinp >= 32 ? ((size_t)(ci / 32) * taps + tap) * 32 + ci % 32 : (size_t)tap * cinp + ci;
                    out[(size_t)co * kpad + k] = L.transposed
                        ? L.w[(((size_t)ci * L.cout + co) * L.k + (L.k - 1 - ky)) * L.k + (L.k - 1 - kx)]
                        : L.w[(((size_t)co * L.cin + ci) * L.k + ky) * L.k + kx];
                }
}

struct Tuning {
    bool no_fold = diag_env("FAV_NO_FOLD") != nullptr;
    bool no_c8 = diag_env("FAV_NO_C8") != nullptr;
    bool no_c8d = diag_env("FAV_NO_C8D") != nullptr;
    bool no_first = diag_env("FAV_NO_FIRST") != nullptr;
    bool no_s2w = diag_env("FAV_NO_S2W") != nullptr;
    bool no_up2 = diag_env("FAV_NO_UP2") != nullptr;
    bool no_wino = diag_env("FAV_NO_WINO") != nullptr;
    bool no_h3 = diag_env("FAV_NO_H3") != nullptr;
    bool no_s2 = diag_env("FAV_NO_S2") != nullptr;
    bool first_1d = diag_env("FAV_FIRST_1D") != nullptr;
    bool wino_f2 = diag_env("FAV_WINO_F2") != nullptr;
    bool no_acc_stats = diag_env("FAV_NO_ACC_STATS") != nullptr;
    bool no_lazy_join = diag_env("FAV_NO_LAZY_JOIN") != nullptr;
    bool lazy_join = diag_env("FAV_LAZY_JOIN") != nullptr;
    int side_sk = diag_env("FAV_SIDE_SK") ? atoi(diag_env("FAV_SIDE_SK")) : 0;
};
const Tuning& tuning() { static const Tuning t; return t; }

ConvKernel select_conv(const Layer& L, const DevConvW& d, int stages, int ups, int precision, bool is_final, int IH, int IW, const Tuning& t)
{
    if (is_final) return !t.no_fold && d.packed[CK_FOLD] && conv_fold_launchable(d.cinp, L.k, L.pad, ups, IH, IW) ? CK_FOLD : CK_GENERIC;
    if (L.transposed) return CK_GENERIC;
    const bool c8 = !t.no_c8 && conv_c8_eligible(d.cinp, d.coutp, L.k, L.stride, stages, ups);
    if (!t.no_first && !t.no_c8d) {
        if (c8 && d.packed[CK_FIRST1D] && conv_c8d_eligible(d.cinp, L.cin, d.coutp, L.k, L.stride, stages, ups))
            return d.packed[CK_FIRST2D] && !t.first_1d ? CK_FIRST2D : CK_FIRST1D;
        if (!c8 && d.packed[CK_FIRST2D] && conv_first2d_eligible(d.cinp, L.cin, d.coutp, L.k, L.stride, stages, ups)) return CK_FIRST2D;
    }
    if (d.packed[CK_S2W] && !t.no_s2w && conv3s2w_eligible(d.cinp, L.cout, d.coutp, L.k, L.stride, L.pad, stages, ups)) return CK_S2W;
    if (d.packed[CK_UP2] && precision == 0 && !t.no_up2 &&
        conv3_up2_eligible(d.cinp, L.cout, d.coutp, L.k, L.stride, L.pad, stages, ups)) return CK_UP2;
    if (precision == 0 && !t.no_wino) {
        if (d.packed[CK_WINO4] && conv3_wino4_eligible(d.cinp, L.cout, d.coutp, L.k, L.stride, L.pad, stages, ups)) return CK_WINO4;
        if (d.packed[CK_WINO] && conv3_wino_eligible(d.cinp, L.cout, d.coutp, L.k, L.stride, L.pad, stages, ups)) return CK_WINO;
    }
    if (c8) return !t.no_c8d && d.packed[CK_C8D] && conv_c8d_eligible(d.cinp, L.cin, d.coutp, L.k, L.stride, stages, ups) ? CK_C8D : CK_C8;
    if (!t.no_h3 && conv3_halo_eligible(d.cinp, d.coutp, L.k, L.stride)) return CK_HALO3;
    if (!t.no_s2 && conv3s2_eligible(d.cinp, d.coutp, L.k, L.stride, stages, ups)) return CK_S2HALO;
    return CK_GENERIC;
}

struct ConvFacts { int tiles; bool counts; int id; };
ConvFacts conv_facts(ConvKernel k, int OH, int OW, int coutp, int precision, bool join)
{
    switch (k) {
    case CK_GENERIC: return {conv_mblocks(OH, OW), false, coutp % 128 == 0 ? 128 : (coutp % 64 == 0 ? 64 : 32)};
    case CK_FOLD:    return {0, false, 1};
    case CK_C8:      return {conv_c8_tiles(OH, OW), true, 8};
    case CK_C8D:     return {conv_c8_tiles(OH, OW), true, 7};
    case CK_FIRST1D: return {conv_first_tiles(OH, OW), true, 6};
    case CK_FIRST2D: return {conv_first2d_tiles(OH, OW), true, 16};
    case CK_S2W:     return {conv3s2w_tiles(OH, OW, coutp), true, 700 + coutp};
    case CK_UP2:     return {conv3_up2_tiles(OH, OW), true, 500 + coutp};
    case CK_WINO:    return {conv3_wino_tiles(OH, OW), true, 400 + coutp + (join ? 1 : 0)};
    case CK_WINO4:   return {conv3_wino4_tiles(OH, OW), true, 600 + coutp + (join ? 1 : 0)};
    case CK_HALO3:   return {conv3_halo_tiles(OH, OW, precision == 0), true, 300 + coutp};
    case CK_S2HALO:  return {conv3s2_tiles(OH, OW), true, 200 + coutp};
    }
    return {0, false, 0};
}

int launch_selected(ConvKernel k, const ConvLaunch& cs, const ConvLaunch& cg, const DevConvW& d, int cin_real, int* counts, hipStream_t st)
{
    const float* w = d.packed[k];
    switch (k) {
    case CK_GENERIC: return launch_conv(cg, st);
    case CK_FOLD:    return launch_conv_fold(cs, w, st);
    case CK_C8:      return launch_conv_c8(cs, counts, st);
    case CK_C8D:     return launch_conv_c8d(cs, cin_real, w, counts, st);
    case CK_FIRST1D: return launch_conv_first(cs, cin_real, w, counts, st);
    case CK_FIRST2D: return launch_conv_first2d(cs, cin_real, w, counts, st);
    case CK_S2W:     return launch_conv3s2w(cs, w, counts, st);
    case CK_UP2:     return launch_conv3_up2(cs, w, counts, st);
    case CK_WINO:    return launch_conv3_wino(cs, w, counts, st);
    case CK_WINO4:   return launch_conv3_wino4(cs, w, counts, st);
    case CK_HALO3:   return launch_conv3_halo(cg, counts, st);
    case CK_S2HALO:  return launch_conv3s2(tuning().side_sk == 2 ? cs : cg, counts, st);
    }
    set_error("internal: unknown convolution kernel %d", (int)k); return FAV_EINVAL;
}

struct InputState { int stages, ups; };
constexpr InputState IN_PLAIN{0, 0};
constexpr InputState IN_NORM{1, 0};
constexpr InputState IN_NORM_UP2{1, 1};

bool pack_weights(ConvKernel k, const Layer& L, const DevConvW& d, std::vector<float>& out)
{
    if (L.transposed) return false;
    const float* w = L.w.data();
    const bool first = conv_c8d_eligible(d.cinp, L.cin, d.coutp, L.k, L.stride, IN_PLAIN.stages, IN_PLAIN.ups);
    const bool full_k = L.cin == d.cinp;
    switch (k) {
    case CK_GENERIC: case CK_C8: case CK_HALO3: case CK_S2HALO:
        return false;
    case CK_C8D:
        if (!first) return false;
        conv_c8d_pack(w, L.cin, L.cout, out); return true;
    case CK_FIRST1D:
        if (!first) return false;
        conv_first_pack(w, L.cin, L.cout, out); return true;
    case CK_FIRST2D:
        if (first) { conv_first2d_pack(w, L.cin, L.cout, out); return true; }
        if (!conv_first2d_eligible(d.cinp, L.cin, d.coutp, L.k, L.stride, IN_PLAIN.stages, IN_PLAIN.ups)) return false;
        conv_first2d_pack_groups(w, L.cin, L.cout, d.coutp, out); return true;
    case CK_WINO:
        if (!full_k || !conv3_wino_eligible(d.cinp, L.cout, d.coutp, L.k, L.stride, L.pad, IN_PLAIN.stages, IN_PLAIN.ups)) return false;
        conv_wino_pack(w, L.cin, L.cout, out); return true;
    case CK_WINO4:
        if (!full_k || tuning().wino_f2 || !conv3_wino4_eligible(d.cinp, L.cout, d.coutp, L.k, L.stride, L.pad, IN_PLAIN.stages, IN_PLAIN.ups)) return false;
        conv_wino4_pack_groups(w, L.cin, L.cout, out); return true;
    case CK_UP2:
        if (!full_k || !conv3_up2_eligible(d.cinp, L.cout, d.coutp, L.k, L.stride, L.pad, IN_NORM_UP2.stages, IN_NORM_UP2.ups)) return false;
        if (L.cout == 64) {
            std::vector<float> w9;
            conv_up2_pack(w, L.cin, out);
            conv_up2w_pack(w, L.cin, w9);
            out.insert(out.end(), w9.begin(), w9.end());
        } else conv_up2w_pack_groups(w, L.cin, L.cout, out);
        return true;
    case CK_S2W:
        if (!full_k || !conv3s2w_eligible(d.cinp, L.cout, d.coutp, L.k, L.stride, L.pad, IN_NORM.stages, IN_NORM.ups)) return false;
        conv_s2w_pack_groups(w, L.cin, L.cout, out); return true;
    case CK_FOLD:
        if (!conv_fold_eligible(d.cinp, L.cout, L.k, L.stride)) return false;
        conv_fold_pack(w, L.cin, d.cinp, L.cout, L.k, out); return true;
    }
    return false;
}

int append_stage(Affine& a, const float* scale, const float* shift, int relu)
{
    if (a.stages >= 2) { set_error("network: more than two stacked normalisations on one tensor are unsupported"); return FAV_EUNSUPPORTED; }
    if (a.stages == 0) { a.scale1 = scale; a.shift1 = shift; a.relu1 = relu; }
    else { a.scale2 = scale; a.shift2 = shift; a.relu2 = relu; }
    ++a.stages;
    return FAV_OK;
}

bool only_tail(const std::vector<Layer>& ls, size_t from, bool& has_tanh, float& mul);
int pow2_ceil(int c) { int p = 4; while (p < c) p <<= 1; return p; }

int pad_channel_counts(std::vector<Layer>& ls, int& chan, int& real, bool& seen_conv, bool top)
{
    for (size_t li = 0; li < ls.size(); ++li) {
        Layer& L = ls[li];
        if (L.type == L_CONV) {
            const bool first_input = !seen_conv && L.cin <= 8;
            seen_conv = true;
            const int cin_new = first_input ? L.cin : chan;
            bool has_tanh = false; float mul = 1.f;
            const bool is_final = top && L.cout == 3 && only_tail(ls, li + 1, has_tanh, mul) && has_tanh;
            const int cout_new = is_final ? L.cout : pow2_ceil(L.cout);
            if (!first_input && L.cin != real) { set_error("network: conv expects %d input channels, its producer has %d", L.cin, real); return FAV_EFORMAT; }
            const int cout_real = L.cout;
            if (cin_new != L.cin || cout_new != L.cout) {
                std::vector<float> w((size_t)cout_new * cin_new * L.k * L.k, 0.f);
                const size_t kk = (size_t)L.k * L.k;
                for (int co = 0; co < L.cout; ++co)
                    for (int ci = 0; ci < L.cin; ++ci) {
                        const float* src = L.transposed ? &L.w[((size_t)ci * L.cout + co) * kk] : &L.w[((size_t)co * L.cin + ci) * kk];
                        float* dst = L.transposed ? &w[((size_t)ci * cout_new + co) * kk] : &w[((size_t)co * cin_new + ci) * kk];
                        std::copy(src, src + kk, dst);
                    }
                L.w.swap(w);
                if (!L.b.empty()) L.b.resize((size_t)cout_new, 0.f);
                L.cin = cin_new; L.cout = cout_new;
            }
            chan = L.cout; real = cout_real;
        } else if (L.type == L_IN) {
            if ((int)L.gamma.size() != real) { set_error("network: InstanceNormalization(%zu) after %d channels", L.gamma.size(), real); return FAV_EFORMAT; }
            L.gamma.resize((size_t)chan, 0.f); L.beta.resize((size_t)chan, 0.f);
        } else if (L.type == L_BN) {
            if ((int)L.mean.size() != real) { set_error("network: SpatialBatchNormalization(%zu) after %d channels", L.mean.size(), real); return FAV_EFORMAT; }
            L.gamma.resize((size_t)chan, 0.f); L.beta.resize((size_t)chan, 0.f); L.mean.resize((size_t)chan, 0.f); L.var.resize((size_t)chan, 1.f);
        } else if (L.type == L_RES) {
            int c = chan, r = real;
            int rc = pad_channel_counts(L.block, c, r, seen_conv, false); if (rc) return rc;
            if (c != chan || r != real) { set_error("network: residual branch changes the channel count"); return FAV_EUNSUPPORTED; }
        }
    }
    return FAV_OK;
}

long long count_params(const std::vector<Layer>& ls)
{
    long long n = 0;
    for (const Layer& L : ls) {
        if (L.type == L_CONV) n += (long long)L.w.size() + (long long)L.b.size();
        else if (L.type == L_IN) n += 2 * (long long)L.gamma.size();
        else if (L.type == L_BN) n += 4 * (long long)L.mean.size();
        else if (L.type == L_RES) n += count_params(L.block);
    }
    return n;
}

bool only_tail(const std::vector<Layer>& ls, size_t from, bool& has_tanh, float& mul)
{
    has_tanh = false; mul = 1.f;
    for (size_t i = from; i < ls.size(); ++i) {
        if (ls[i].type == L_TANH) { if (has_tanh) return false; has_tanh = true; }
        else if (ls[i].type == L_MUL) { if (!has_tanh) return false; mul *= ls[i].mul; }
        else if (ls[i].type != L_IDENTITY) return false;
    }
    return true;
}

}

struct fav_net {
    int device = 0;
    std::vector<Layer> layers;
    std::vector<Layer> exec;
    int pad = 0;
    bool pad_folded = false;
    int in_channels = 0;
    long long params = 0;
    std::vector<DevConvW> convs;
    std::vector<DevIN> ins;
    float* ones = nullptr; float* zeros = nullptr;
    float* sk_ws = nullptr; unsigned* sk_flags = nullptr; unsigned sk_epoch = 0;
    float* ks_ws = nullptr; int* ks_cnt = nullptr;
    struct LazyOut { bool active = false; int pitch = 0, rows = 0, shave = 0, conv_index = -1; } lazy;
    unsigned* sk_err_host = nullptr; unsigned* sk_err_dev = nullptr;
    bool shared_device = false;
    int precision = 0;
    int acc_parity = 0;
    bool acc_dirty = false;
    bool branch_tail_acc_ok = false;
    int reserve_cus = 0;
    int curH = 0, curW = 0;
    std::vector<DevBuf> bufs;
    std::vector<void*> slabs; char* slab_cur = nullptr; size_t slab_left = 0;
    size_t cursor = 0, conv_cursor = 0, in_cursor = 0;
    hipStream_t st = nullptr;
    float* stage = nullptr; size_t stage_bytes = 0;
    bool profiling = false;
    struct ProfRec { hipEvent_t a, b; int conv; };
    std::vector<ProfRec> prof_pending;
    std::vector<double> prof_ms, prof_macs; std::vector<int> prof_n, prof_tile;

    ~fav_net()
    {
        (void)hipSetDevice(device);
        (void)hipFree(stage);
        for (auto& c : convs) { (void)hipFree(c.wgt); (void)hipFree(c.bias); (void)hipFree(c.wgt16); for (float* p : c.packed) (void)hipFree(p); }
        for (auto& i : ins) { (void)hipFree(i.gamma); (void)hipFree(i.beta); (void)hipFree(i.scale); (void)hipFree(i.shift); (void)hipFree(i.acc); }
        for (void* sp : slabs) (void)hipFree(sp);
        (void)hipFree(ones); (void)hipFree(zeros); (void)hipFree(sk_ws); (void)hipFree(sk_flags); (void)hipFree(ks_ws); (void)hipFree(ks_cnt); if (sk_err_host) (void)hipHostFree(sk_err_host);
    }
    int upload_layers(std::vector<Layer>& ls, int& chan_pitch, int& maxc);
    int upload();
    int alloc(size_t bytes, float** out);
    int timed_conv(const ConvLaunch& c, int conv_index, const Layer& L, ConvKernel kernel, int* counts);
    int run(std::vector<Layer>& ls, Act& cur, bool top, float* out_planar, float* out_raw);
    bool res_block_is_winograd(const Layer& R, size_t first_conv) const;
    bool acc_stats_ok(const std::vector<Layer>& ls, size_t li) const;
    int forward_padded(const float* in8, int H, int W, float* out_planar, float* out_raw, hipStream_t stream);
    int forward_padded_unordered(const float* in8, int H, int W, float* out_planar, float* out_raw, hipStream_t stream);
    void out_size(int H, int W, int* Ho, int* Wo) const;
};

int fav_net::upload_layers(std::vector<Layer>& ls, int& chan_pitch, int& maxc)
{
    for (Layer& L : ls) {
        if (L.type == L_CONV) {
            convs.emplace_back();
            DevConvW& d = convs.back();
            d.cinp = chan_pitch;
            if (L.cin > chan_pitch || (chan_pitch != 8 && L.cin != chan_pitch)) {
                set_error("network: conv expects %d input channels, producer has %d", L.cin, chan_pitch); return FAV_EFORMAT; }
            if (L.k < 1 || L.stride < 1 || L.pad < 0) { set_error("network: bad convolution geometry"); return FAV_EFORMAT; }
            if ((d.cinp & (d.cinp - 1)) != 0) {
                set_error("network: a convolution with %d input channels is unsupported (channel counts must be powers of two)", d.cinp);
                return FAV_EUNSUPPORTED; }
            d.coutp = (L.cout + 31) / 32 * 32;
            d.kpad = (L.k * L.k * d.cinp + 31) / 32 * 32;
            std::vector<float> w;
            repack_weights(L, d.cinp, d.coutp, d.kpad, w);
            int rc = dev_upload(w, 0, &d.wgt); if (rc) return rc;
            rc = dev_upload(L.b, (size_t)d.coutp, &d.bias); if (rc) return rc;
            if (!L.transposed && conv3_halo_eligible(d.cinp, d.coutp, L.k, L.stride)) {
                std::vector<unsigned short> w16(w.size());
                for (size_t i = 0; i < w.size(); ++i) { unsigned b; memcpy(&b, &w[i], 4); w16[i] = (unsigned short)((b + 0x7FFFu + ((b >> 16) & 1u)) >> 16); }
                FAV_HIP(hipMalloc(reinterpret_cast<void**>(&d.wgt16), w16.size() * 2));
                FAV_HIP(hipMemcpy(d.wgt16, w16.data(), w16.size() * 2, hipMemcpyHostToDevice));
            }
            if (L.transposed && (L.stride != 2 || L.adj != 1 || L.pad > L.k - 1)) {
                set_error("network: SpatialFullConvolution is supported for stride 2, adj 1 (models_video.lua:99-102), got s=%d adj=%d", L.stride, L.adj);
                return FAV_EUNSUPPORTED; }
            std::vector<float> wk;
            for (int k = 0; k < CONV_KERNELS; ++k)
                if (pack_weights((ConvKernel)k, L, d, wk)) { rc = dev_upload(wk, 0, &d.packed[k]); if (rc) return rc; }
            chan_pitch = L.cout;
            maxc = std::max(maxc, std::max(d.coutp, d.cinp));
        } else if (L.type == L_IN) {
            if ((int)L.gamma.size() != chan_pitch) { set_error("network: InstanceNormalization(%zu) after %d channels", L.gamma.size(), chan_pitch); return FAV_EFORMAT; }
            ins.emplace_back();
            DevIN& d = ins.back();
            int rc = dev_upload(L.gamma, 0, &d.gamma); if (rc) return rc;
            rc = dev_upload(L.beta, 0, &d.beta); if (rc) return rc;
            FAV_HIP(hipMalloc(reinterpret_cast<void**>(&d.scale), L.gamma.size() * sizeof(float)));
            FAV_HIP(hipMalloc(reinterpret_cast<void**>(&d.shift), L.gamma.size() * sizeof(float)));
            d.acc_bytes = 2 * stat_acc_words((int)L.gamma.size()) * sizeof(long long);
            FAV_HIP(hipMalloc(reinterpret_cast<void**>(&d.acc), d.acc_bytes));
            FAV_HIP(hipMemset(d.acc, 0, d.acc_bytes));
        } else if (L.type == L_BN) {
            if ((int)L.mean.size() != chan_pitch) { set_error("network: SpatialBatchNormalization(%zu) after %d channels", L.mean.size(), chan_pitch); return FAV_EFORMAT; }
            std::vector<float> sc(L.mean.size()), sh(L.mean.size());
            for (size_t i = 0; i < sc.size(); ++i) {
                const double s = (double)L.gamma[i] / std::sqrt((double)L.var[i] + (double)L.eps);
                sc[i] = (float)s; sh[i] = (float)((double)L.beta[i] - (double)L.mean[i] * s);
            }
            ins.emplace_back();
            DevIN& d = ins.back();
            int rc = dev_upload(sc, 0, &d.scale); if (rc) return rc;
            rc = dev_upload(sh, 0, &d.shift); if (rc) return rc;
        } else if (L.type == L_RES) {
            int cp = chan_pitch;
            int rc = upload_layers(L.block, cp, maxc); if (rc) return rc;
            if (cp != chan_pitch) { set_error("network: residual branch changes the channel count"); return FAV_EUNSUPPORTED; }
        }
    }
    return FAV_OK;
}

int fav_net::upload()
{
    FAV_HIP(hipSetDevice(device));
    if (layers.empty()) { set_error("network: empty model"); return FAV_EFORMAT; }
    pad = 0; pad_folded = false;
    if (layers[0].type == L_PAD) {
        const Layer& P = layers[0];
        if (P.pad_mode == 0 && P.pl == P.pr && P.pl == P.pt && P.pl == P.pb) { pad = P.pl; pad_folded = true; }
    }
    in_channels = 0;
    for (const Layer& L : layers) if (L.type == L_CONV) { in_channels = L.cin; break; }
    if (in_channels != 7 && in_channels != 3) {
        set_error("network: first convolution has %d input channels; video models take 7 (models_video.lua:57), image models 3", in_channels);
        return FAV_EUNSUPPORTED; }
    exec = layers;
    int chan0 = 8;
    int real0 = in_channels; bool seen_conv = false;
    int rc = pad_channel_counts(exec, chan0, real0, seen_conv, true); if (rc) return rc;
    int chan = 8, maxc = 8;
    rc = upload_layers(exec, chan, maxc); if (rc) return rc;
    params = count_params(layers);
    std::vector<float> o((size_t)maxc, 1.f), z((size_t)maxc, 0.f);
    rc = dev_upload(o, 0, &ones); if (rc) return rc;
    rc = dev_upload(z, 0, &zeros); if (rc) return rc;
    FAV_HIP(hipMalloc(reinterpret_cast<void**>(&sk_ws), conv_streamk_workspace_bytes()));
    FAV_HIP(hipMalloc(reinterpret_cast<void**>(&sk_flags), conv_streamk_grid() * sizeof(unsigned)));
    FAV_HIP(hipMemset(sk_flags, 0, conv_streamk_grid() * sizeof(unsigned)));
    FAV_HIP(hipMalloc(reinterpret_cast<void**>(&ks_ws), conv3_wino4_ksplit_bytes()));
    FAV_HIP(hipMalloc(reinterpret_cast<void**>(&ks_cnt), 256 * sizeof(int)));
    FAV_HIP(hipMemset(ks_cnt, 0, 256 * sizeof(int)));
    FAV_HIP(hipHostMalloc(reinterpret_cast<void**>(&sk_err_host), sizeof(unsigned), hipHostMallocMapped));
    *sk_err_host = 0;
    FAV_HIP(hipHostGetDevicePointer(reinterpret_cast<void**>(&sk_err_dev), sk_err_host, 0));
    return FAV_OK;
}

int fav_net::alloc(size_t bytes, float** out)
{
    bytes = (bytes + 255) / 256 * 256;
    if (cursor < bufs.size()) {
        if (bufs[cursor].bytes < bytes) { set_error("internal: activation arena mismatch"); return FAV_EINVAL; }
        *out = static_cast<float*>(bufs[cursor++].p);
        return FAV_OK;
    }
    if (slab_left < bytes) {
        const size_t sz = std::max(bytes, (size_t)256 << 20);
        void* sp = nullptr;
        FAV_HIP(hipMalloc(&sp, sz));
        slabs.push_back(sp); slab_cur = static_cast<char*>(sp); slab_left = sz;
    }
    DevBuf b; b.bytes = bytes; b.p = slab_cur;
    slab_cur += bytes; slab_left -= bytes;
    bufs.push_back(b); ++cursor;
    *out = static_cast<float*>(b.p);
    return FAV_OK;
}

int fav_net::timed_conv(const ConvLaunch& c, int conv_index, const Layer& L, ConvKernel kernel, int* counts)
{
    if (c.pre.acc1 != nullptr && kernel != CK_WINO4) { set_error("internal: accumulator-form InstanceNorm in front of a kernel that cannot take it"); return FAV_EINVAL; }
    ConvLaunch cs = c;
    cs.reserve_cus = reserve_cus;
    cs.no_sk = shared_device ? 1 : 0;
    cs.sk_ws = sk_ws; cs.sk_flags = sk_flags; cs.sk_epoch = ++sk_epoch;
    cs.sk_err = sk_err_dev;
    cs.ks_ws = ks_ws; cs.ks_cnt = ks_cnt;
    if (sk_epoch == 0xffffffffu) sk_epoch = 0;
    ConvLaunch cg = cs;
    if (reserve_cus > 0 && tuning().side_sk != 1) cg.no_sk = 1;
    auto go = [&]() { return launch_selected(kernel, cs, cg, convs[conv_index], L.cin, counts, st); };
    char tag[96] = "";
    if (TraceRange::enabled()) snprintf(tag, sizeof tag, "fav:conv%d k%d s%d %d->%d %dx%d", conv_index, L.k, L.stride, L.cin, L.cout, c.OW, c.OH);
    TraceRange tr(tag);
    if (!profiling) return go();
    ProfRec r; r.conv = conv_index;
    FAV_HIP(hipEventCreateWithFlags(&r.a, hipEventDisableSystemFence)); FAV_HIP(hipEventCreateWithFlags(&r.b, hipEventDisableSystemFence));
    FAV_HIP(hipEventRecord(r.a, st));
    int rc = go();
    FAV_HIP(hipEventRecord(r.b, st));
    prof_pending.push_back(r);
    if ((int)prof_ms.size() <= conv_index) { prof_ms.resize(conv_index + 1, 0.0); prof_macs.resize(conv_index + 1, 0.0); prof_n.resize(conv_index + 1, 0); prof_tile.resize(conv_index + 1, 0); }
    prof_macs[conv_index] = (double)c.OH * c.OW * L.cout * L.cin * L.k * L.k;
    prof_tile[conv_index] = conv_facts(kernel, c.OH, c.OW, c.COUTp, precision, c.join_skip != nullptr).id;
    return rc;
}

static int count_convs(const std::vector<Layer>& ls)
{
    int n = 0;
    for (const Layer& l : ls) { if (l.type == L_CONV) ++n; else if (l.type == L_RES) n += count_convs(l.block); }
    return n;
}

bool fav_net::acc_stats_ok(const std::vector<Layer>& ls, size_t li) const
{
    if (tuning().no_acc_stats) return false;
    if (li + 3 >= ls.size() || ls[li + 1].type != L_IN || ls[li + 2].type != L_RELU || ls[li + 3].type != L_CONV) return false;
    if (conv_cursor >= convs.size()) return false;
    const Layer& c2 = ls[li + 3]; const DevConvW& d2 = convs[conv_cursor];
    return select_conv(c2, d2, 1, 0, precision, false, 0, 0, tuning()) == CK_WINO4;
}

bool fav_net::res_block_is_winograd(const Layer& R, size_t first_conv) const
{
    const std::vector<Layer>& b = R.block;
    if (b.size() != 5 || b[0].type != L_CONV || b[1].type != L_IN || b[2].type != L_RELU || b[3].type != L_CONV || b[4].type != L_IN) return false;
    if (first_conv + 1 >= convs.size()) return false;
    for (int k = 0; k < 2; ++k) {
        const Layer& c = b[k ? 3 : 0]; const DevConvW& d = convs[first_conv + (size_t)k];
        const ConvKernel kernel = select_conv(c, d, 1, 0, precision, false, 0, 0, tuning());
        if ((kernel != CK_WINO && kernel != CK_WINO4) || d.packed[CK_WINO] == nullptr) return false;
    }
    return true;
}

int fav_net::run(std::vector<Layer>& ls, Act& cur, bool top, float* out_planar, float* out_raw)
{
    for (size_t li = 0; li < ls.size(); ++li) {
        Layer& L = ls[li];
        switch (L.type) {
        case L_PAD: {
            if (top && li == 0 && pad_folded) break;
            if (cur.data == nullptr || cur.join_skip != nullptr) { set_error("network: misplaced padding layer"); return FAV_EUNSUPPORTED; }
            if (L.pad_mode == 0 && (std::max(L.pl, L.pr) >= cur.W() || std::max(L.pt, L.pb) >= cur.H())) { set_error("network: reflection padding %d %d %d %d of a %dx%d tensor", L.pl, L.pr, L.pt, L.pb, cur.W(), cur.H()); return FAV_EINVAL; }
            Act nxt;
            nxt.Hp = cur.H() + L.pt + L.pb; nxt.Wp = cur.W() + L.pl + L.pr; nxt.C = cur.C; nxt.pre = cur.pre;
            if (nxt.pre.acc1 != nullptr) { set_error("internal: accumulator-form InstanceNorm in front of a padding layer"); return FAV_EINVAL; }
            int rc = alloc((size_t)nxt.Hp * nxt.Wp * nxt.C * sizeof(float), &nxt.data); if (rc) return rc;
            rc = launch_pad_nhwc(cur.data, cur.Hp, cur.Wp, cur.P(), cur.C, cur.ups, nxt.data, L.pl, L.pr, L.pt, L.pb, L.pad_mode, st); if (rc) return rc;
            cur = nxt;
            break;
        }
        case L_CONV: {
            const DevConvW& d = convs[conv_cursor++];
            if (cur.C != d.cinp) { set_error("internal: channel pitch mismatch (%d vs %d)", cur.C, d.cinp); return FAV_EINVAL; }
            ConvLaunch c;
            c.in = cur.data; c.IH = cur.H(); c.IW = cur.W(); c.IWp = cur.P(); c.ups = cur.ups; c.CIN = d.cinp;
            c.pre = cur.pre;
            c.wgt = d.wgt; c.bias = d.bias; c.COUT = L.cout; c.COUTp = d.coutp; c.KH = c.KW = L.k; c.stride = L.stride;
            c.pad = L.pad; c.Kpad = d.kpad;
            if (L.transposed) {
                if (cur.ups != 0) { set_error("network: SpatialFullConvolution directly after an upsampling is unsupported"); return FAV_EUNSUPPORTED; }
                c.ups = 1; c.stuff = 1; c.IH = 2 * cur.Hp; c.IW = 2 * cur.Wp; c.stride = 1; c.pad = L.k - 1 - L.pad;
                c.OH = c.IH + 2 * c.pad - L.k + 1; c.OW = c.IW + 2 * c.pad - L.k + 1;
            } else {
                c.OH = (c.IH + 2 * L.pad - L.k) / L.stride + 1;
                c.OW = (c.IW + 2 * L.pad - L.k) / L.stride + 1;
            }
            if (c.IH + 2 * c.pad < L.k || c.IW + 2 * c.pad < L.k) { set_error("network: input too small for the architecture"); return FAV_EINVAL; }
            bool has_tanh = false; float mul = 1.f;
            const bool is_final = top && only_tail(ls, li + 1, has_tanh, mul) && has_tanh && L.cout == 3;
            const ConvKernel kernel = select_conv(L, d, cur.pre.stages, cur.ups, precision, is_final, c.IH, c.IW, tuning());
            Act nxt;
            nxt.Hp = c.OH; nxt.Wp = c.OW; nxt.C = L.cout;
            if (is_final && L.transposed) { set_error("network: a transposed convolution as the last layer is unsupported"); return FAV_EUNSUPPORTED; }
            if (is_final) {
                c.final_mode = 1; c.tanh_mul = mul; c.out_planar = out_planar; c.out_raw_nchw = out_raw;
                int rc = timed_conv(c, (int)conv_cursor - 1, L, kernel, nullptr); if (rc) return rc;
                cur = nxt;
                return FAV_OK;
            }
            if (L.cout % 4 != 0) { set_error("network: %d output channels (must be a multiple of 4 except for the last layer)", L.cout); return FAV_EUNSUPPORTED; }
            const bool pitched_out = lazy.active && (int)conv_cursor - 1 == lazy.conv_index;
            int rc;
            if (pitched_out) {
                if (c.OH != lazy.rows - 2 * lazy.shave || c.OW > lazy.pitch - 2 * lazy.shave) { set_error("internal: pending residual join of mismatching shapes"); return FAV_EINVAL; }
                float* base = nullptr;
                rc = alloc((size_t)lazy.rows * lazy.pitch * L.cout * sizeof(float), &base); if (rc) return rc;
                nxt.data = base + ((size_t)lazy.shave * lazy.pitch + lazy.shave) * L.cout; nxt.pitch = lazy.pitch; c.OWp = lazy.pitch;
            } else { rc = alloc((size_t)c.OH * c.OW * L.cout * sizeof(float), &nxt.data); if (rc) return rc; }
            const bool want_stats = li + 1 < ls.size() && ls[li + 1].type == L_IN;
            const ConvFacts facts = conv_facts(kernel, c.OH, c.OW, d.coutp, precision, cur.join_skip != nullptr);
            nxt.mblocks = facts.tiles; nxt.ppitch = d.coutp;
            const bool acc = kernel == CK_WINO4 && want_stats && !pitched_out && cur.join_skip == nullptr &&
                             (acc_stats_ok(ls, li) || (branch_tail_acc_ok && !top && li + 2 == ls.size() && !tuning().no_acc_stats && precision == 0));
            if (acc) {
                DevIN& din = ins[in_cursor];
                nxt.acc = din.acc + (size_t)acc_parity * stat_acc_words(L.cout); nxt.acc_other = din.acc + (size_t)(acc_parity ^ 1) * stat_acc_words(L.cout);
                c.stat_acc = nxt.acc;
            }
            if (want_stats && !acc) { rc = alloc((size_t)nxt.mblocks * d.coutp * 2 * sizeof(float), &nxt.partials); if (rc) return rc; }
            if (want_stats && !acc && facts.counts) { float* cp = nullptr; rc = alloc((size_t)nxt.mblocks * sizeof(int), &cp); if (rc) return rc; nxt.counts = reinterpret_cast<int*>(cp); }
            c.out = nxt.data; c.partials = nxt.partials;
            if (cur.join_skip != nullptr || pitched_out) {
                if (kernel != CK_WINO && kernel != CK_WINO4) { set_error("internal: a pending residual join next to a convolution that is not the Winograd kernel's"); return FAV_EINVAL; }
                c.join_skip = cur.join_skip; c.join_out = cur.join_out;
            }
            if (kernel == CK_HALO3 && precision == 1) c.wgt16 = d.wgt16;
            int* counts = facts.counts ? (nxt.counts ? nxt.counts : reinterpret_cast<int*>(zeros)) : nullptr;
            rc = timed_conv(c, (int)conv_cursor - 1, L, kernel, counts); if (rc) return rc;
            cur = nxt;
            break;
        }
        case L_IN: {
            const DevIN& d = ins[in_cursor++];
            const int C = (int)L.gamma.size();
            const int M = cur.Hp * cur.Wp;
            if (cur.data == nullptr || C != cur.C) { set_error("network: misplaced InstanceNormalization"); return FAV_EUNSUPPORTED; }
            if (cur.acc != nullptr && cur.pre.stages == 0) {
                cur.pre = Affine();
                cur.pre.acc1 = cur.acc; cur.pre.acc1_zero = cur.acc_other; cur.pre.gamma1 = d.gamma; cur.pre.beta1 = d.beta; cur.pre.eps1 = L.eps; cur.pre.count1 = M;
                cur.pre.relu1 = 0; cur.pre.stages = 1;
            } else if (cur.partials != nullptr && cur.pre.stages == 0) {
                int rc = launch_in_finalize(cur.partials, cur.counts, cur.mblocks, M, CONV_BM, C, cur.ppitch, d.gamma, d.beta, L.eps,
                                            d.scale, d.shift, st);
                if (rc) return rc;
                rc = append_stage(cur.pre, d.scale, d.shift, 0); if (rc) return rc;
            } else {
                Affine normalised = cur.pre;
                int rc = append_stage(normalised, d.scale, d.shift, 0); if (rc) return rc;
                float* part = nullptr;
                const int mb = (M + 127) / 128;
                rc = alloc((size_t)mb * C * 2 * sizeof(float), &part); if (rc) return rc;
                rc = launch_stats(cur.data, M, C, cur.pre, part, st); if (rc) return rc;
                rc = launch_in_finalize(part, nullptr, mb, M, 128, C, C, d.gamma, d.beta, L.eps, d.scale, d.shift, st); if (rc) return rc;
                cur.pre = normalised;
            }
            cur.partials = nullptr; cur.counts = nullptr; cur.acc = nullptr; cur.acc_other = nullptr;
            break;
        }
        case L_BN: {
            const DevIN& d = ins[in_cursor++];
            if (cur.data == nullptr || (int)L.mean.size() != cur.C) { set_error("network: misplaced SpatialBatchNormalization"); return FAV_EUNSUPPORTED; }
            int rc = append_stage(cur.pre, d.scale, d.shift, 0); if (rc) return rc;
            cur.partials = nullptr; cur.counts = nullptr;
            break;
        }
        case L_RELU:
            if (cur.pre.stages == 0) (void)append_stage(cur.pre, ones, zeros, 1);
            else if (cur.pre.stages == 1) cur.pre.relu1 = 1;
            else cur.pre.relu2 = 1;
            cur.partials = nullptr;
            break;
        case L_UP:
            if (L.scale != 2 || cur.ups != 0) { set_error("network: only a single x2 nearest upsampling per convolution is supported"); return FAV_EUNSUPPORTED; }
            cur.ups = 1;
            break;
        case L_RES: {
            if (cur.ups != 0) { set_error("network: residual block directly after an upsampling is unsupported"); return FAV_EUNSUPPORTED; }
            Act skip = cur;
            Act br = cur;
            br.partials = nullptr;
            int rc;
            if (cur.join_skip != nullptr) {
                float* zb = nullptr;
                rc = alloc((size_t)cur.Hp * cur.P() * cur.C * sizeof(float), &zb); if (rc) return rc;
                br.join_out = zb;
                skip = Act(); skip.data = zb; skip.Hp = cur.Hp; skip.Wp = cur.Wp; skip.C = cur.C; skip.pitch = cur.P();
            }
            const int nconv = count_convs(L.block);
            const bool lazy_out = !tuning().no_lazy_join && (tuning().wino_f2 || tuning().lazy_join) && precision == 0 &&
                                  li + 1 < ls.size() && ls[li + 1].type == L_RES && skip.pre.stages == 0 && skip.ups == 0 &&
                                  res_block_is_winograd(L, conv_cursor) && res_block_is_winograd(ls[li + 1], conv_cursor + (size_t)nconv);
            if (lazy_out) { lazy.active = true; lazy.pitch = skip.P(); lazy.rows = skip.Hp; lazy.shave = L.shave; lazy.conv_index = (int)conv_cursor + nconv - 1; }
            size_t nx = li + 1;
            if (nx < ls.size() && ls[nx].type == L_UP && ls[nx].scale == 2) ++nx;
            const bool join_stats = nx < ls.size() && ls[nx].type == L_IN;
            branch_tail_acc_ok = !lazy_out && !join_stats;
            rc = run(L.block, br, false, nullptr, nullptr);
            lazy.active = false; branch_tail_acc_ok = false;
            if (rc) return rc;
            if (br.pre.stages != 1 || br.pre.relu1 || br.ups != 0) { set_error("network: residual branch must end in conv + InstanceNormalization"); return FAV_EUNSUPPORTED; }
            if (br.Hp != skip.Hp - 2 * L.shave || br.Wp != skip.Wp - 2 * L.shave || br.C != skip.C) {
                set_error("network: residual branch output %dx%d does not match the shaved skip %dx%d", br.Wp, br.Hp,
                          skip.Wp - 2 * L.shave, skip.Hp - 2 * L.shave);
                return FAV_EUNSUPPORTED; }
            if (lazy_out) {
                cur = br;
                cur.partials = nullptr; cur.counts = nullptr;
                cur.join_skip = skip.data + ((size_t)L.shave * skip.P() + L.shave) * skip.C; cur.join_out = nullptr;
                break;
            }
            Act z; z.Hp = br.Hp; z.Wp = br.Wp; z.C = br.C;
            rc = alloc((size_t)z.Hp * z.Wp * z.C * sizeof(float), &z.data); if (rc) return rc;
            if (join_stats) {
                z.mblocks = res_add_stat_blocks(z.Hp, z.Wp); z.ppitch = z.C;
                rc = alloc((size_t)z.mblocks * z.C * 2 * sizeof(float), &z.partials); if (rc) return rc;
                float* cp = nullptr; rc = alloc((size_t)z.mblocks * sizeof(int), &cp); if (rc) return rc; z.counts = reinterpret_cast<int*>(cp);
            }
            rc = launch_res_add(br.data, br.pre.scale1, br.pre.shift1, skip.data, skip.Hp, skip.Wp, L.shave, skip.pre, z.C,
                                z.data, z.partials, z.counts, st, skip.P(), &br.pre);
            if (rc) return rc;
            cur = z;
            break;
        }
        case L_TANH: case L_MUL:
            set_error("network: Tanh/MulConstant are only supported after the last convolution"); return FAV_EUNSUPPORTED;
        case L_IDENTITY: break;
        }
    }
    if (top) { set_error("network: the model does not end in a 3-channel convolution followed by Tanh"); return FAV_EUNSUPPORTED; }
    return FAV_OK;
}

void fav_net::out_size(int H, int W, int* Ho, int* Wo) const
{
    int h = H + 2 * pad, w = W + 2 * pad;
    std::function<void(const std::vector<Layer>&)> walk = [&](const std::vector<Layer>& ls) {
        for (const Layer& L : ls) {
            if (L.type == L_PAD) { if (&L == &layers[0] && pad_folded) continue; h += L.pt + L.pb; w += L.pl + L.pr; }
            else if (L.type == L_CONV && L.transposed) { h = (h - 1) * L.stride - 2 * L.pad + L.k + L.adj; w = (w - 1) * L.stride - 2 * L.pad + L.k + L.adj; }
            else if (L.type == L_CONV) { h = (h + 2 * L.pad - L.k) / L.stride + 1; w = (w + 2 * L.pad - L.k) / L.stride + 1; }
            else if (L.type == L_UP) { h *= L.scale; w *= L.scale; }
            else if (L.type == L_RES) walk(L.block);
        }
    };
    walk(layers);
    *Ho = h; *Wo = w;
}

namespace {
struct DeviceOrder { std::mutex mu; hipStream_t last = nullptr; bool valid = false; };
DeviceOrder& device_order(int device)
{
    static DeviceOrder order[64];
    return order[(device >= 0 && device < 64) ? device : 0];
}
}

static void forget_stream(int device, hipStream_t stream)
{
    DeviceOrder& ord = device_order(device);
    std::lock_guard<std::mutex> order_lock(ord.mu);
    if (ord.valid && ord.last == stream) { (void)hipStreamSynchronize(stream); ord.valid = false; ord.last = nullptr; }
}

extern "C" int fav_net_forget_stream(fav_net* net, fav_hipstream_t stream)
{
    FAV_REQUIRE(net, "fav_net_forget_stream: null network");
    FAV_HIP(hipSetDevice(net->device));
    forget_stream(net->device, static_cast<hipStream_t>(stream));
    return FAV_OK;
}

int fav_net::forward_padded(const float* in8, int H, int W, float* out_planar, float* out_raw, hipStream_t stream)
{
    FAV_HIP(hipSetDevice(device));
    DeviceOrder& ord = device_order(device);
    std::lock_guard<std::mutex> order_lock(ord.mu);
    if (ord.valid && ord.last != stream && hipStreamSynchronize(ord.last) != hipSuccess)
        (void)hipGetLastError();
    ord.valid = true; ord.last = stream;
    return forward_padded_unordered(in8, H, W, out_planar, out_raw, stream);
}

int fav_net::forward_padded_unordered(const float* in8, int H, int W, float* out_planar, float* out_raw, hipStream_t stream)
{
    if (sk_err_host && *reinterpret_cast<volatile unsigned*>(sk_err_host)) {
        *sk_err_host = 0;
        shared_device = true;
        set_error("a stream-K hand-off between convolution blocks timed out in an earlier launch of this network: its result was "
                  "wrong (two networks running concurrently on one device? see the concurrency note in fav.h)");
        return FAV_EHIP;
    }
    if (H != curH || W != curW) {
        if (!bufs.empty()) {
            FAV_HIP(hipDeviceSynchronize());
            for (void* sp : slabs) (void)hipFree(sp);
            slabs.clear(); slab_cur = nullptr; slab_left = 0;
            bufs.clear();
        }
        curH = H; curW = W;
    }
    st = stream; cursor = 0; conv_cursor = 0; in_cursor = 0;
    if (acc_dirty) {
        for (DevIN& i : ins) if (i.acc) FAV_HIP(hipMemsetAsync(i.acc, 0, i.acc_bytes, stream));
        acc_dirty = false;
    }
    if (precision == 0 && !tuning().no_acc_stats && !tuning().no_wino) acc_parity ^= 1;
    Act cur;
    cur.data = const_cast<float*>(in8); cur.Hp = H + 2 * pad; cur.Wp = W + 2 * pad; cur.C = 8;
    const int rc = run(exec, cur, true, out_planar, out_raw);
    if (rc) acc_dirty = true;
    return rc;
}

static int finish_create(fav_net* net, fav_net** out)
{
    int rc = net->upload();
    if (rc) { delete net; return rc; }
    *out = net;
    return FAV_OK;
}

extern "C" int fav_net_create(const char* t7_path_host, int device, fav_net** out)
{
    FAV_REQUIRE(t7_path_host && out, "fav_net_create: null argument");
    int rc = ensure_device(); if (rc) return rc;
    FAV_ABI_TRY
    std::unique_ptr<fav_net> net(new fav_net());
    net->device = device;
    rc = t7_parse_model(t7_path_host, net->layers);
    if (rc) return rc;
    return finish_create(net.release(), out);
    FAV_ABI_CATCH("fav_net_create")
}

extern "C" int fav_net_pack_host(const char* t7_path_host, void* blob_host, size_t capacity, size_t* bytes)
{
    FAV_REQUIRE(t7_path_host && bytes, "fav_net_pack_host: null argument");
    FAV_ABI_TRY
    std::vector<Layer> layers;
    int rc = t7_parse_model(t7_path_host, layers); if (rc) return rc;
    std::vector<uint8_t> blob;
    rc = blob_pack(layers, blob); if (rc) return rc;
    *bytes = blob.size();
    if (blob_host) {
        FAV_REQUIRE(capacity >= blob.size(), "fav_net_pack_host: capacity %zu < %zu", capacity, blob.size());
        memcpy(blob_host, blob.data(), blob.size());
    }
    return FAV_OK;
    FAV_ABI_CATCH("fav_net_pack_host")
}

extern "C" int fav_net_create_from_blob(const void* blob_host, size_t bytes, int device, fav_net** out)
{
    FAV_REQUIRE(blob_host && out, "fav_net_create_from_blob: null argument");
    int rc = ensure_device(); if (rc) return rc;
    FAV_ABI_TRY
    std::unique_ptr<fav_net> net(new fav_net());
    net->device = device;
    rc = blob_unpack(blob_host, bytes, net->layers);
    if (rc) return rc;
    return finish_create(net.release(), out);
    FAV_ABI_CATCH("fav_net_create_from_blob")
}

extern "C" void fav_net_destroy(fav_net* net) { delete net; }

extern "C" int fav_net_check(fav_net* net)
{
    FAV_REQUIRE(net, "fav_net_check: null net");
    if (net->sk_err_host && *reinterpret_cast<volatile unsigned*>(net->sk_err_host)) {
        *net->sk_err_host = 0;
        net->shared_device = true;
        set_error("a stream-K hand-off between convolution blocks timed out: the frame(s) computed since the last check are wrong "
                  "(another context holding compute units of this device? see the concurrency note in fav.h); this network now runs "
                  "with data-parallel grids (fav_net_set_shared_device)");
        return FAV_EHIP;
    }
    return FAV_OK;
}

extern "C" int fav_net_set_shared_device(fav_net* net, int shared)
{
    FAV_REQUIRE(net, "fav_net_set_shared_device: null net");
    net->shared_device = shared != 0;
    return FAV_OK;
}

extern "C" int fav_net_describe_host(const fav_net* net, char* buf_host, size_t capacity)
{
    FAV_REQUIRE(net && buf_host && capacity > 0, "fav_net_describe_host: null argument");
    const std::string s = describe_layers(net->layers);
    FAV_REQUIRE(s.size() + 1 <= capacity, "fav_net_describe_host: need %zu bytes", s.size() + 1);
    memcpy(buf_host, s.c_str(), s.size() + 1);
    return FAV_OK;
}

extern "C" int fav_net_profile_enable(fav_net* net, int on)
{
    FAV_REQUIRE(net, "fav_net_profile_enable: null net");
    net->profiling = on != 0;
    return FAV_OK;
}

extern "C" int fav_net_profile_read_host(fav_net* net, int capacity, int* count, double* ms_sum, int* launches,
                                         double* macs_per_launch, int* ntile)
{
    FAV_REQUIRE(net && count && ms_sum && launches && macs_per_launch && ntile, "fav_net_profile_read_host: null argument");
    FAV_HIP(hipSetDevice(net->device));
    for (auto& r : net->prof_pending) {
        FAV_HIP(hipEventSynchronize(r.b));
        float ms = 0.f;
        FAV_HIP(hipEventElapsedTime(&ms, r.a, r.b));
        net->prof_ms[r.conv] += ms; net->prof_n[r.conv] += 1;
        (void)hipEventDestroy(r.a); (void)hipEventDestroy(r.b);
    }
    net->prof_pending.clear();
    const int n = (int)net->prof_ms.size();
    FAV_REQUIRE(n <= capacity, "fav_net_profile_read_host: need capacity %d", n);
    for (int i = 0; i < n; ++i) { ms_sum[i] = net->prof_ms[i]; launches[i] = net->prof_n[i]; macs_per_launch[i] = net->prof_macs[i]; ntile[i] = net->prof_tile[i]; }
    *count = n;
    std::fill(net->prof_ms.begin(), net->prof_ms.end(), 0.0); std::fill(net->prof_n.begin(), net->prof_n.end(), 0);
    return FAV_OK;
}

extern "C" int fav_t7_describe_host(const char* t7_path_host, char* buf_host, size_t capacity)
{
    FAV_REQUIRE(t7_path_host && buf_host && capacity > 0, "fav_t7_describe_host: null argument");
    FAV_ABI_TRY
    std::vector<Layer> layers;
    int rc = t7_parse_model(t7_path_host, layers); if (rc) return rc;
    const std::string s = describe_layers(layers);
    FAV_REQUIRE(s.size() + 1 <= capacity, "fav_t7_describe_host: need %zu bytes", s.size() + 1);
    memcpy(buf_host, s.c_str(), s.size() + 1);
    return FAV_OK;
    FAV_ABI_CATCH("fav_t7_describe_host")
}

extern "C" long long fav_net_param_count(const fav_net* net) { return net ? net->params : 0; }

extern "C" int fav_net_output_size(const fav_net* net, int H, int W, int* Ho, int* Wo)
{
    FAV_REQUIRE(net && Ho && Wo && H > 0 && W > 0, "fav_net_output_size: bad argument");
    net->out_size(H, W, Ho, Wo);
    return FAV_OK;
}

extern "C" int fav_net_forward(fav_net* net, const float* in7, float* out3, int H, int W, fav_hipstream_t stream)
{
    FAV_REQUIRE(net && in7 && out3 && H > 0 && W > 0, "fav_net_forward: bad argument");
    FAV_REQUIRE(net->pad < H && net->pad < W, "fav_net_forward: %dx%d is smaller than the reflection padding %d", W, H, net->pad);
    FAV_HIP(hipSetDevice(net->device));
    hipStream_t st = static_cast<hipStream_t>(stream);
    const size_t bytes = (size_t)(H + 2 * net->pad) * (W + 2 * net->pad) * 8 * sizeof(float);
    if (net->stage_bytes < bytes) {
        FAV_HIP(hipDeviceSynchronize());
        (void)hipFree(net->stage); net->stage = nullptr; net->stage_bytes = 0;
        FAV_HIP(hipMalloc(reinterpret_cast<void**>(&net->stage), bytes));
        net->stage_bytes = bytes;
    }
    float* in8 = net->stage;
    int rc = launch_nchw_to_nhwc_pad(in7, net->in_channels, H, W, net->pad, 8, in8, st); if (rc) return rc;
    return net->forward_padded(in8, H, W, nullptr, out3, st);
}

extern "C" int fav_conv2d_nchw_f32(const float* in, int Cin, int H, int W, const float* weight, const float* bias, int Cout,
                                   int k, int stride, int pad, const float* gamma, const float* beta, float eps, int relu,
                                   float* out, fav_hipstream_t stream)
{
    FAV_REQUIRE(in && weight && out && Cin > 0 && Cout > 0 && k > 0 && stride > 0 && pad >= 0, "fav_conv2d_nchw_f32: bad argument");
    int rc = ensure_device(); if (rc) return rc;
    hipStream_t st = static_cast<hipStream_t>(stream);
    const int cinp = (Cin + 3) / 4 * 4, coutp = (Cout + 31) / 32 * 32, kpad = (k * k * cinp + 31) / 32 * 32;
    const int OH = (H + 2 * pad - k) / stride + 1, OW = (W + 2 * pad - k) / stride + 1;
    FAV_REQUIRE(OH > 0 && OW > 0, "fav_conv2d_nchw_f32: empty output");
    const int M = OH * OW, mb = conv_mblocks(OH, OW);
    Layer L; L.cin = Cin; L.cout = Cout; L.k = k;
    L.w.resize((size_t)Cin * Cout * k * k);
    FAV_HIP(hipMemcpy(L.w.data(), weight, L.w.size() * sizeof(float), hipMemcpyDeviceToHost));
    std::vector<float> wre, hb((size_t)coutp, 0.f);
    repack_weights(L, cinp, coutp, kpad, wre);
    if (bias) FAV_HIP(hipMemcpy(hb.data(), bias, (size_t)Cout * sizeof(float), hipMemcpyDeviceToHost));
    float *dw = nullptr, *db = nullptr, *din = nullptr, *dout = nullptr, *dpart = nullptr, *dsc = nullptr, *dsh = nullptr;
    auto cleanup = [&]() { (void)hipFree(dw); (void)hipFree(db); (void)hipFree(din); (void)hipFree(dout); (void)hipFree(dpart); (void)hipFree(dsc); (void)hipFree(dsh); };
    rc = dev_upload(wre, 0, &dw); if (rc) { cleanup(); return rc; }
    rc = dev_upload(hb, 0, &db); if (rc) { cleanup(); return rc; }
    if (hipMalloc(reinterpret_cast<void**>(&din), (size_t)H * W * cinp * 4) != hipSuccess ||
        hipMalloc(reinterpret_cast<void**>(&dout), (size_t)M * Cout * 4) != hipSuccess ||
        hipMalloc(reinterpret_cast<void**>(&dpart), (size_t)mb * coutp * 8) != hipSuccess ||
        hipMalloc(reinterpret_cast<void**>(&dsc), (size_t)coutp * 4) != hipSuccess ||
        hipMalloc(reinterpret_cast<void**>(&dsh), (size_t)coutp * 4) != hipSuccess) { cleanup(); return hip_fail(hipErrorOutOfMemory, "hipMalloc"); }
    rc = launch_nchw_to_nhwc_pad(in, Cin, H, W, 0, cinp, din, st);
    ConvLaunch c;
    c.in = din; c.IH = H; c.IW = W; c.IWp = W; c.CIN = cinp; c.wgt = dw; c.bias = db; c.COUT = Cout; c.COUTp = coutp;
    c.KH = c.KW = k; c.stride = stride; c.pad = pad; c.Kpad = kpad; c.OH = OH; c.OW = OW; c.out = dout;
    c.partials = gamma ? dpart : nullptr;
    if (!rc) rc = launch_conv(c, st);
    Affine t;
    if (!rc && gamma) {
        rc = launch_in_finalize(dpart, nullptr, mb, M, CONV_BM, Cout, coutp, gamma, beta, eps, dsc, dsh, st);
        t.scale1 = dsc; t.shift1 = dsh; t.relu1 = relu; t.stages = 1;
    }
    if (!rc) rc = launch_nhwc_to_nchw(dout, M, Cout, t, out, st);
    if (hipStreamSynchronize(st) != hipSuccess && !rc) rc = hip_fail(hipGetLastError(), "fav_conv2d_nchw_f32");
    cleanup();
    return rc;
}

extern "C" int fav_net_set_precision(fav_net* net, int mode)
{
    FAV_REQUIRE(net && (mode == 0 || mode == 1), "fav_net_set_precision: mode must be FAV_PRECISION_FP32 or FAV_PRECISION_BF16_OPERANDS");
    if (net->precision != mode) { net->curH = -1; net->acc_dirty = true; }
    net->precision = mode;
    return FAV_OK;
}

namespace fav {
int net_device(const fav_net* n) { return n->device; }
int net_pad(const fav_net* n) { return n->pad; }
int net_in_channels(const fav_net* n) { return n->in_channels; }
void net_out_size(const fav_net* n, int H, int W, int* Ho, int* Wo) { n->out_size(H, W, Ho, Wo); }
int net_forward_padded(fav_net* n, const float* in8, int H, int W, float* out_planar, hipStream_t st) { return n->forward_padded(in8, H, W, out_planar, nullptr, st); }
void net_forget_stream(const fav_net* n, hipStream_t st) { forget_stream(n->device, st); }
void net_reserve_cus(fav_net* n, int cus) { n->reserve_cus = std::max(n->reserve_cus, cus); }
}
```

Before: 657.7.

## Fuse residual join into final branch Winograd conv via grid-wide stats barrier

When the residual branch's last conv runs as a single-round Winograd-4 launch with accumulated instance-norm stats, each block now waits on a global arrival counter until all blocks have contributed stats. It then computes scale and shift, applies the normalisation, adds the skip tensor and stores the joined result directly. This removes the separate residual-add kernel and the raw conv-output round trip through memory. In exchange it adds an in-kernel spin barrier that requires every block to be co-resident, a timeout error path, and extra arena reset logic.

```diff
diff --git a/fast-artistic-videos_amd/csrc/fav_internal.h b/fast-artistic-videos_amd/csrc/fav_internal.h
--- a/fast-artistic-videos_amd/csrc/fav_internal.h
+++ b/fast-artistic-videos_amd/csrc/fav_internal.h
@@ -98,6 +98,46 @@
 {
     return hi_sum >= STAT_NONFINITE / 2 || hi_sum <= -(STAT_NONFINITE / 2) || hi_squares >= STAT_NONFINITE / 2 || hi_squares <= -(STAT_NONFINITE / 2);
 }
+
+#ifdef __HIPCC__
+template <bool FRESH = false>
+__device__ __forceinline__ void stat_acc_scale_shift(const long long* acc, int C, int i, int count, const float* gamma, const float* beta, float eps,
+                                                     float& scale, float& shift)
+{
+    long long w0 = 0, w1 = 0, w2 = 0, w3 = 0;
+    if (FRESH) {
+        long long v[STAT_COPIES][4];
+#pragma unroll
+        for (int cp = 0; cp < STAT_COPIES; ++cp)
+#pragma unroll
+            for (int q = 0; q < 4; ++q) v[cp][q] = __hip_atomic_load(acc + ((size_t)cp * C + i) * 4 + q, __ATOMIC_RELAXED, __HIP_MEMORY_SCOPE_AGENT);
+#pragma unroll
+        for (int cp = 0; cp < STAT_COPIES; ++cp) { w0 += v[cp][0]; w1 += v[cp][1]; w2 += v[cp][2]; w3 += v[cp][3]; }
+    } else {
+#pragma unroll
+        for (int cp = 0; cp < STAT_COPIES; ++cp) {
+            const longlong2* a = reinterpret_cast<const longlong2*>(acc + ((size_t)cp * C + i) * 4);
+            const longlong2 lo = a[0], hi = a[1];
+            w0 += lo.x; w1 += lo.y; w2 += hi.x; w3 += hi.y;
+        }
+    }
+    const double s1 = ((double)w1 * 4294967296.0 + (double)w0) * (1.0 / 1099511627776.0);
+    const double s2 = ((double)w3 * 4294967296.0 + (double)w2) * (1.0 / 1099511627776.0);
+    const double mean = s1 / (double)count;
+    double var = s2 / (double)count - mean * mean;
+    var = var > 0.0 ? var : 0.0;
+    const double sc = stat_acc_poisoned(w1, w3) ? (double)NAN : (double)gamma[i] / sqrt(var + (double)eps);
+    scale = (float)sc; shift = (float)((double)beta[i] - mean * sc);
+}
+__device__ __forceinline__ void stat_acc_zero(long long* acc, int C, int i)
+{
+#pragma unroll
+    for (int cp = 0; cp < STAT_COPIES; ++cp) {
+        longlong2* z = reinterpret_cast<longlong2*>(acc + ((size_t)cp * C + i) * 4);
+        z[0] = longlong2{0, 0}; z[1] = longlong2{0, 0};
+    }
+}
+#endif
 
 struct ConvLaunch {
     const float* in = nullptr;
@@ -127,6 +167,9 @@
     const float* join_skip = nullptr; float* join_out = nullptr; int OWp = 0;
     long long* stat_acc = nullptr;
     float* ks_ws = nullptr; int* ks_cnt = nullptr;
+    const float* fj_skip = nullptr; int fj_pitch = 0;
+    long long* fj_acc_zero = nullptr; const float* fj_gamma = nullptr; const float* fj_beta = nullptr; float fj_eps = 0.f;
+    unsigned* fj_cnt = nullptr; unsigned fj_target = 0;
 };
 inline size_t conv3_wino4_ksplit_bytes() { return (size_t)256 * 2 * 256 * 128 * sizeof(float); }
 size_t conv_streamk_workspace_bytes();
@@ -159,6 +202,7 @@
 int launch_conv3_wino(const ConvLaunch& p, const float* wpk, int* counts, hipStream_t st);
 bool conv3_wino4_eligible(int cin_pitch, int cout, int coutp, int k, int stride, int pad, int stages, int ups);
 int conv3_wino4_tiles(int OH, int OW);
+int conv3_wino4_grid(int OH, int OW, int cout, int reserve_cus, bool have_ks, bool* one_round);
 int launch_conv3_wino4(const ConvLaunch& p, const float* wpk, int* counts, hipStream_t st);
 bool conv3_up2_eligible(int cin_pitch, int cout, int coutp, int k, int stride, int pad, int stages, int ups);
 int conv3_up2_tiles(int OH, int OW);
diff --git a/fast-artistic-videos_amd/csrc/kernels_elem.hip b/fast-artistic-videos_amd/csrc/kernels_elem.hip
--- a/fast-artistic-videos_amd/csrc/kernels_elem.hip
+++ b/fast-artistic-videos_amd/csrc/kernels_elem.hip
@@ -128,27 +128,8 @@
     __shared__ float ss[ACC ? 2048 : 4];
     if (ACC) {
         for (int i = threadIdx.x; i < C; i += 256) {
-            long long w0 = 0, w1 = 0, w2 = 0, w3 = 0;
-#pragma unroll
-            for (int cp = 0; cp < STAT_COPIES; ++cp) {
-                const longlong2* a = reinterpret_cast<const longlong2*>(br.acc1 + ((size_t)cp * C + i) * 4);
-                const longlong2 lo = a[0], hi = a[1];
-                w0 += lo.x; w1 += lo.y; w2 += hi.x; w3 += hi.y;
-            }
-            const double s1 = ((double)w1 * 4294967296.0 + (double)w0) * (1.0 / 1099511627776.0);
-            const double s2 = ((double)w3 * 4294967296.0 + (double)w2) * (1.0 / 1099511627776.0);
-            const double mean = s1 / (double)br.count1;
-            double var = s2 / (double)br.count1 - mean * mean;
-            var = var > 0.0 ? var : 0.0;
-            const double sc = stat_acc_poisoned(w1, w3) ? (double)NAN : (double)br.gamma1[i] / sqrt(var + (double)br.eps1);
-            ss[i] = (float)sc; ss[C + i] = (float)((double)br.beta1[i] - mean * sc);
-            if (blockIdx.x == 0) {
-#pragma unroll
-                for (int cp = 0; cp < STAT_COPIES; ++cp) {
-                    longlong2* zz = reinterpret_cast<longlong2*>(br.acc1_zero + ((size_t)cp * C + i) * 4);
-                    zz[0] = longlong2{0, 0}; zz[1] = longlong2{0, 0};
-                }
-            }
+            stat_acc_scale_shift(br.acc1, C, i, br.count1, br.gamma1, br.beta1, br.eps1, ss[i], ss[C + i]);
+            if (blockIdx.x == 0) stat_acc_zero(br.acc1_zero, C, i);
         }
         __syncthreads();
         scale = ss; shift = ss + C;
diff --git a/fast-artistic-videos_amd/csrc/kernels_wino4.hip b/fast-artistic-videos_amd/csrc/kernels_wino4.hip
--- a/fast-artistic-videos_amd/csrc/kernels_wino4.hip
+++ b/fast-artistic-videos_amd/csrc/kernels_wino4.hip
@@ -38,6 +38,8 @@
     long long* dbg;
     long long* stat_acc; const long long* acc1; long long* acc1_zero; const float* gamma1; const float* beta1; float eps1; int count1;
     int COUT, groups;
+    const float* fj_skip; int fj_pitch; long long* fj_acc_zero; const float* fj_gamma; const float* fj_beta; float fj_eps;
+    unsigned* fj_cnt; unsigned fj_target; unsigned* sk_err;
 };
 
 __device__ __forceinline__ void w4_store16_wt(void* ptr, v4f v)
@@ -73,9 +75,12 @@
     y[3] = w4_fma(3.375f, d2, w4_fma(0.421875f, d1, m[5]));
 }
 
-template <int MODE, int VAR = 0, bool WIDE = false>
+template <int MODE_, int VAR = 0, bool WIDE = false>
 __global__ __launch_bounds__(512) __attribute__((amdgpu_waves_per_eu(2, 2))) void conv3_wino4_kernel(const Wino4Args p)
 {
+    constexpr bool FJ = MODE_ >= 3;
+    constexpr int MODE = FJ ? MODE_ - 3 : MODE_;
+    static_assert(MODE_ <= 4 && (!FJ || (!WIDE && VAR == 0)), "the producer-side join: one 128-filter group, a plain input or a pending normalisation");
     constexpr bool AFF = MODE != 0, JOIN = MODE == 2;
     constexpr bool PAIR = (VAR & 8) == 0 && MODE != 2;
     constexpr int NT = 512;
@@ -101,27 +106,8 @@
     }
     if (MODE == 1 && p.acc1 != nullptr) {
         for (int i = t; i < CIN; i += NT) {
-            long long w0 = 0, w1 = 0, w2 = 0, w3 = 0;
-#pragma unroll
-            for (int cp = 0; cp < STAT_COPIES; ++cp) {
-                const longlong2* a = reinterpret_cast<const longlong2*>(p.acc1 + ((size_t)cp * CIN + i) * 4);
-                const longlong2 lo = a[0], hi = a[1];
-                w0 += lo.x; w1 += lo.y; w2 += hi.x; w3 += hi.y;
-            }
-            const double s1 = ((double)w1 * 4294967296.0 + (double)w0) * (1.0 / 1099511627776.0);
-            const double s2 = ((double)w3 * 4294967296.0 + (double)w2) * (1.0 / 1099511627776.0);
-            const double mean = s1 / (double)p.count1;
-            double var = s2 / (double)p.count1 - mean * mean;
-            var = var > 0.0 ? var : 0.0;
-            const double sc = stat_acc_poisoned(w1, w3) ? (double)NAN : (double)p.gamma1[i] / sqrt(var + (double)p.eps1);
-            aff[i] = (float)sc; aff[CIN + i] = (float)((double)p.beta1[i] - mean * sc);
-            if (blockIdx.x == 0) {
-#pragma unroll
-                for (int cp = 0; cp < STAT_COPIES; ++cp) {
-                    longlong2* z = reinterpret_cast<longlong2*>(p.acc1_zero + ((size_t)cp * CIN + i) * 4);
-                    z[0] = longlong2{0, 0}; z[1] = longlong2{0, 0};
-                }
-            }
+            stat_acc_scale_shift(p.acc1, CIN, i, p.count1, p.gamma1, p.beta1, p.eps1, aff[i], aff[CIN + i]);
+            if (blockIdx.x == 0) stat_acc_zero(p.acc1_zero, CIN, i);
         }
     } else if (AFF) for (int i = t; i < CIN; i += NT) { aff[i] = p.scale1[i]; aff[CIN + i] = p.shift1[i]; }
     const float lo1 = (MODE == 1 && p.relu1) ? 0.f : -INFINITY;
@@ -398,7 +384,7 @@
                 for (int r = 0; r < 4; ++r)
 #pragma unroll
                     for (int b = 0; b < 4; ++b) {
-                        __builtin_amdgcn_raw_buffer_store_b32(__builtin_bit_cast(int, y[a][b][r]), ors, ro + r * 4 * cpb + b * cpb, 0, 0);
+                        if (!FJ) __builtin_amdgcn_raw_buffer_store_b32(__builtin_bit_cast(int, y[a][b][r]), ors, ro + r * 4 * cpb + b * cpb, 0, 0);
                         sm += y[a][b][r];
                     }
             }
@@ -421,7 +407,7 @@
                 for (int c = 0; c < 16; ++c) {
                     if (c < ncols) {
                         const float v = y[a][c & 3][c >> 2];
-                        __builtin_amdgcn_raw_buffer_store_b32(__builtin_bit_cast(int, v), ors, ro + c * cpb, 0, 0);
+                        if (!FJ) __builtin_amdgcn_raw_buffer_store_b32(__builtin_bit_cast(int, v), ors, ro + c * cpb, 0, 0);
                         sm += rv ? v : 0.f;
                     }
                 }
@@ -456,10 +442,53 @@
             } else if (g == 0) p.partials[(size_t)u * (WIDE ? p.COUT : 128) + cb] = make_float2(mu, m2);
         }
         if (p.partials != nullptr && p.stat_acc == nullptr && t == 0 && grp == 0) p.counts[u] = nv;
+        if (FJ) {
+            asm volatile("s_waitcnt vmcnt(0)" ::: "memory");
+            __syncthreads();
+            if (t == 0) __hip_atomic_fetch_add(p.fj_cnt, 1u, __ATOMIC_RELAXED, __HIP_MEMORY_SCOPE_AGENT);
+            const __amdgpu_buffer_rsrc_t krs = __builtin_amdgcn_make_buffer_rsrc(const_cast<float*>(p.fj_skip), 0, ((p.OH - 1) * p.fj_pitch + p.OW) * 512, 0x00020000);
+            float k[4][4][4];
+#pragma unroll
+            for (int a = 0; a < 4; ++a) {
+                const int ko = oyb + a < p.OH ? ((oyb + a) * p.fj_pitch + ox0) * 512 + cb * 4 : (int)0xFFFF0000;
+#pragma unroll
+                for (int c = 0; c < 16; ++c) {
+                    k[a][c & 3][c >> 2] = 0.f;
+                    if (inside || c < ncols)
+                        k[a][c & 3][c >> 2] = __builtin_bit_cast(float, __builtin_amdgcn_raw_buffer_load_b32(krs, ko + c * 512, 0, 0));
+                }
+            }
+            asm volatile("" ::: "memory"); __builtin_amdgcn_sched_barrier(0);
+            DBG_T();
+            if (t == 0) {
+                unsigned spins = 0;
+                while ((int)(__hip_atomic_load(p.fj_cnt, __ATOMIC_RELAXED, __HIP_MEMORY_SCOPE_AGENT) - p.fj_target) < 0) {
+                    __builtin_amdgcn_s_sleep(4);
+                    if (++spins > (1u << 22)) { if (p.sk_err) __hip_atomic_store(p.sk_err, 1u, __ATOMIC_RELAXED, __HIP_MEMORY_SCOPE_SYSTEM); break; }
+                }
+            }
+            __syncthreads();
+            __builtin_amdgcn_fence(__ATOMIC_ACQUIRE, "agent");
+            DBG_T();
+            float fsc, fsh;
+            int cbo = cb; asm volatile("" : "+v"(cbo));
+            stat_acc_scale_shift<true>(p.stat_acc, 128, cbo, p.OH * p.OW, p.fj_gamma, p.fj_beta, p.fj_eps, fsc, fsh);
+            if (blockIdx.x == 0 && t < 128) { int tz = t; asm volatile("" : "+v"(tz)); stat_acc_zero(p.fj_acc_zero, 128, tz); }
+#pragma unroll
+            for (int a = 0; a < 4; ++a) {
+                const int ro = oyb + a < p.OH ? ((oyb + a) * p.OWp + ox0) * cpb + cb * 4 : (int)0xFFFF0000;
+#pragma unroll
+                for (int c = 0; c < 16; ++c)
+                    if (inside || c < ncols) {
+                        const float z = fmaf(y[a][c & 3][c >> 2], fsc, fsh) + k[a][c & 3][c >> 2];
+                        __builtin_amdgcn_raw_buffer_store_b32(__builtin_bit_cast(int, z), ors, ro + c * cpb, 0, 0);
+                    }
+            }
+        }
         DBG_T();
     };
     const int units = WIDE ? upix * p.groups : upix;
-    if (!p.stream) {
+    if (FJ || !p.stream) {
         for (int u = lb; u < units; u += gridDim.x) work(u, 0, nslices, -1, 0);
     } else {
         const long long tot = (long long)units * nslices;
@@ -478,59 +507,80 @@
 #undef DBG_T
 }
 
-void wino4_debug_report(const long long* hbuf, int grid, int mode)
+void wino4_debug_report(const long long* hbuf, int grid, int mode, bool fj)
 {
     long long t0 = hbuf[0];
     for (int b = 0; b < grid; ++b) t0 = std::min(t0, hbuf[b * 24]);
-    double sum[4] = {0, 0, 0, 0}, tend = 0, ck = 0, wk = 0; int items = 0;
+    const int per = fj ? 7 : 5;
+    double sum[4] = {0, 0, 0, 0}, tend = 0, ck = 0, wk = 0, wait_sum = 0, wait_max = 0, arrive_last = 0; int items = 0;
     for (int b = 0; b < grid; ++b) {
         const long long* r = &hbuf[b * 24]; const int n = (int)r[23];
-        for (int i = 1; i + 4 < n + 1 && i + 4 <= 20; i += 5) {
-            for (int q = 0; q < 4; ++q) sum[q] += (r[i + q + 1] - r[i + q]) * 0.01;
-            ++items; tend = std::max(tend, (r[i + 4] - t0) * 0.01);
+        for (int i = 1; i + per - 1 < n + 1 && i + per - 1 <= 20; i += per) {
+            for (int q = 0; q < 3; ++q) sum[q] += (r[i + q + 1] - r[i + q]) * 0.01;
+            sum[3] += (r[i + per - 1] - r[i + 3]) * 0.01;
+            if (fj) {
+                const double w = (r[i + 5] - r[i + 4]) * 0.01;
+                wait_sum += w; wait_max = std::max(wait_max, w); arrive_last = std::max(arrive_last, (r[i + 4] - t0) * 0.01);
+            }
+            ++items; tend = std::max(tend, (r[i + per - 1] - t0) * 0.01);
         }
         ck += r[21]; wk += r[22];
     }
     fprintf(stderr, "WINO4DBG mode=%d grid=%d units=%d  K loop: %.3f GHz;  per unit: prologue %.2f  loop %.2f  epilogue %.2f us;  last block ends at %.2f us\n",
             mode, grid, items, wk ? ck / (wk * 10.0) : 0.0, items ? sum[0] / items : 0.0, items ? sum[1] / items : 0.0, items ? sum[3] / items : 0.0, tend);
-}
-
-template <int MODE, bool WIDE>
+    if (fj) fprintf(stderr, "WINO4DBG   joining launch: wait for all blocks mean %.2f  max %.2f us (inside the epilogue);  last block arrives at %.2f us\n",
+                    items ? wait_sum / items : 0.0, wait_max, arrive_last);
+}
+
+struct Wino4Plan { int grid, stream, shares; };
+int wino4_plan(int units, int reserve_cus, bool have_ks, Wino4Plan& pl)
+{
+    const int dv = cur_dev();
+    static int cus[MAX_DEVICES] = {};
+    if (!cus[dv]) FAV_HIP(hipDeviceGetAttribute(&cus[dv], hipDeviceAttributeMultiprocessorCount, dv));
+    static const bool no_stream = diag_env("FAV_W4_NO_STREAM") != nullptr;
+    static const int grid_cap = diag_env("FAV_W4_GRID") ? atoi(diag_env("FAV_W4_GRID")) : 0;
+    pl.grid = std::min(units, std::max(1, cus[dv] - reserve_cus));
+    if (grid_cap > 0) pl.grid = std::min(pl.grid, std::max(1, grid_cap));
+    pl.shares = grid_cap > 0 ? std::max(1, std::min(W4_SHARES, grid_cap)) : W4_SHARES;
+    const int rounds = (units + pl.shares - 1) / pl.shares, rem = units - (rounds - 1) * pl.shares;
+    pl.stream = (rounds >= 2 && rem * 5 <= pl.shares * 3 && pl.shares <= W4_MEET_MAX && have_ks && !no_stream) ? 1 : 0;
+    if (pl.stream) pl.grid = std::min(pl.grid, pl.shares);
+    return FAV_OK;
+}
+
+template <int MODE, bool WIDE, bool FJ = false>
 int launch_wino4_t(const Wino4Args& a0, int reserve_cus, hipStream_t st)
 {
 #ifdef FAV_DIAG
     static const int var = diag_env("FAV_W4_VAR") ? atoi(diag_env("FAV_W4_VAR")) : 0;
-    const auto kern = (!WIDE && MODE == 1 && var == 1) ? conv3_wino4_kernel<1, 1> : (!WIDE && MODE == 1 && var == 2) ? conv3_wino4_kernel<1, 2> : (!WIDE && MODE == 1 && var == 3) ? conv3_wino4_kernel<1, 3> :
+    const auto kern = FJ ? conv3_wino4_kernel<MODE != 2 ? MODE + 3 : 3> :
+                      (!WIDE && MODE == 1 && var == 1) ? conv3_wino4_kernel<1, 1> : (!WIDE && MODE == 1 && var == 2) ? conv3_wino4_kernel<1, 2> : (!WIDE && MODE == 1 && var == 3) ? conv3_wino4_kernel<1, 3> :
                       (!WIDE && MODE == 1 && var == 7) ? conv3_wino4_kernel<1, 7> : (!WIDE && MODE == 1 && var == 6) ? conv3_wino4_kernel<1, 6> :
                       (!WIDE && MODE == 2 && var == 16) ? conv3_wino4_kernel<2, 16> :
                       (MODE != 2 && var == 8) ? conv3_wino4_kernel<MODE, MODE != 2 ? 8 : 0, WIDE> : conv3_wino4_kernel<MODE, 0, WIDE>;
-    const bool pair = MODE != 2 && !(var & 8);
+    const bool pair = MODE != 2 && (FJ || !(var & 8));
 #else
-    const auto kern = conv3_wino4_kernel<MODE, 0, WIDE>;
+    const auto kern = FJ ? conv3_wino4_kernel<MODE != 2 ? MODE + 3 : 3> : conv3_wino4_kernel<MODE, 0, WIDE>;
     const bool pair = MODE != 2;
 #endif
     const size_t lds = (size_t)(W4_SMEM + ((MODE == 2 || pair) ? W4_RBUF : 0) + 2 * a0.CIN + 4) * sizeof(float);
     const int dv = cur_dev();
-    static int cus[MAX_DEVICES] = {};
-    if (!cus[dv]) {
+    static bool ready[MAX_DEVICES] = {};
+    if (!ready[dv]) {
         FAV_HIP(hipFuncSetAttribute(reinterpret_cast<const void*>(kern), hipFuncAttributeMaxDynamicSharedMemorySize, 160 * 1024));
-        int occ = 0; int prop_cus = 0;
-        FAV_HIP(hipDeviceGetAttribute(&prop_cus, hipDeviceAttributeMultiprocessorCount, dv));
+        int occ = 0;
         FAV_HIP(hipOccupancyMaxActiveBlocksPerMultiprocessor(&occ, reinterpret_cast<const void*>(kern), 512, lds));
         if (occ < 1) { set_error("winograd F(4x4) conv: kernel does not fit on a CU"); return FAV_EHIP; }
-        cus[dv] = prop_cus;
+        ready[dv] = true;
     }
     const int units = a0.units_x * a0.units_y * (WIDE ? a0.groups : 1);
-    int grid = std::min(units, std::max(1, cus[dv] - reserve_cus));
+    Wino4Plan pl;
+    { const int rc = wino4_plan(units, reserve_cus, a0.ks_ws && a0.ks_cnt, pl); if (rc) return rc; }
+    const int grid = pl.grid;
     Wino4Args a = a0; a.dbg = nullptr;
-    static const bool no_stream = diag_env("FAV_W4_NO_STREAM") != nullptr;
-    static const int grid_cap = diag_env("FAV_W4_GRID") ? atoi(diag_env("FAV_W4_GRID")) : 0;
-    if (grid_cap > 0) grid = std::min(grid, std::max(1, grid_cap));
-    const int shares = grid_cap > 0 ? std::max(1, std::min(W4_SHARES, grid_cap)) : W4_SHARES;
-    const int rounds = (units + shares - 1) / shares, rem = units - (rounds - 1) * shares;
-    a.stream = (rounds >= 2 && rem * 5 <= shares * 3 && shares <= W4_MEET_MAX && a0.ks_ws && a0.ks_cnt && !no_stream) ? 1 : 0;
-    a.shares = shares;
-    if (a.stream) grid = std::min(grid, shares);
+    a.stream = pl.stream; a.shares = pl.shares;
+    if (FJ) FAV_REQUIRE(!a.stream && grid == units && a.stat_acc && a.fj_skip && a.fj_cnt, "winograd F(4x4) conv: a producer-side residual join on a launch of more than one round");
     static int dbg_n = diag_env("FAV_WINO_DBG") ? atoi(diag_env("FAV_WINO_DBG")) : 0;
     static long long* dbuf = nullptr;
     const bool dbg = dbg_n > 0 && --dbg_n == 0;
@@ -540,7 +590,7 @@
     if (dbg) {
         std::vector<long long> hb((size_t)512 * 24);
         FAV_HIP(hipStreamSynchronize(st)); FAV_HIP(hipMemcpy(hb.data(), dbuf, hb.size() * 8, hipMemcpyDeviceToHost));
-        wino4_debug_report(hb.data(), grid, MODE);
+        wino4_debug_report(hb.data(), grid, MODE, FJ);
     }
     return FAV_OK;
 }
@@ -553,6 +603,14 @@
            cout == coutp && cout % 128 == 0 && cout >= 128 && cout <= 1024;
 }
 int conv3_wino4_tiles(int OH, int OW) { return ((OH + 15) / 16) * ((OW + 15) / 16); }
+int conv3_wino4_grid(int OH, int OW, int cout, int reserve_cus, bool have_ks, bool* one_round)
+{
+    const int units = conv3_wino4_tiles(OH, OW) * (cout / 128);
+    Wino4Plan pl;
+    if (wino4_plan(units, reserve_cus, have_ks, pl) != FAV_OK) { if (one_round) *one_round = false; return 0; }
+    if (one_round) *one_round = !pl.stream && pl.grid == units;
+    return pl.grid;
+}
 
 int launch_conv3_wino4(const ConvLaunch& c, const float* wpk, int* counts, hipStream_t st)
 {
@@ -573,6 +631,14 @@
     a.stat_acc = c.stat_acc; a.acc1 = c.pre.acc1; a.acc1_zero = c.pre.acc1_zero; a.gamma1 = c.pre.gamma1; a.beta1 = c.pre.beta1; a.eps1 = c.pre.eps1; a.count1 = c.pre.count1;
     if (c.stat_acc != nullptr && a.partials == nullptr) a.partials = reinterpret_cast<float2*>(c.stat_acc);
     FAV_REQUIRE(c.pre.acc1 == nullptr || (c.join_skip == nullptr && c.pre.stages == 1 && c.pre.count1 > 0), "winograd F(4x4) conv: accumulator-form InstanceNorm on an unsupported input");
+    a.fj_skip = c.fj_skip; a.fj_pitch = c.fj_pitch; a.fj_acc_zero = c.fj_acc_zero; a.fj_gamma = c.fj_gamma; a.fj_beta = c.fj_beta; a.fj_eps = c.fj_eps;
+    a.fj_cnt = c.fj_cnt; a.fj_target = c.fj_target; a.sk_err = c.sk_err;
+    if (c.fj_skip != nullptr) {
+        FAV_REQUIRE(c.join_skip == nullptr && a.groups == 1 && c.stat_acc != nullptr && c.fj_acc_zero != nullptr && c.fj_cnt != nullptr && c.OWp == 0 && c.fj_pitch >= c.OW,
+                    "winograd F(4x4) conv: a producer-side residual join needs one 128-filter group, accumulator statistics and a plain output");
+        FAV_REQUIRE((long long)(c.OH + 1) * c.fj_pitch * 128 < (1ll << 29), "winograd F(4x4) conv: skip tensor too large for 32-bit byte offsets");
+        return c.pre.stages >= 1 ? launch_wino4_t<1, false, true>(a, c.reserve_cus, st) : launch_wino4_t<0, false, true>(a, c.reserve_cus, st);
+    }
     if (c.join_skip != nullptr) {
         FAV_REQUIRE(c.join_out != nullptr && c.pre.stages == 1 && c.pre.relu1 == 0, "winograd F(4x4) conv: a pending residual join needs its output tensor and exactly one pending normalisation");
         FAV_REQUIRE(a.groups == 1, "winograd F(4x4) conv: a pending residual join is formed by 128-filter layers only");
diff --git a/fast-artistic-videos_amd/csrc/net.cpp b/fast-artistic-videos_amd/csrc/net.cpp
--- a/fast-artistic-videos_amd/csrc/net.cpp
+++ b/fast-artistic-videos_amd/csrc/net.cpp
@@ -41,6 +41,7 @@
     int pitch = 0;
     const float* join_skip = nullptr; float* join_out = nullptr;
     long long* acc = nullptr; long long* acc_other = nullptr;
+    bool joined = false;
     int H() const { return Hp << ups; }
     int W() const { return Wp << ups; }
     int P() const { return pitch ? pitch : Wp; }
@@ -87,6 +88,7 @@
     bool no_acc_stats = diag_env("FAV_NO_ACC_STATS") != nullptr;
     bool no_lazy_join = diag_env("FAV_NO_LAZY_JOIN") != nullptr;
     bool lazy_join = diag_env("FAV_LAZY_JOIN") != nullptr;
+    bool no_fused_join = diag_env("FAV_NO_FUSED_JOIN") != nullptr;
     int side_sk = diag_env("FAV_SIDE_SK") ? atoi(diag_env("FAV_SIDE_SK")) : 0;
 };
 const Tuning& tuning() { static const Tuning t; return t; }
@@ -296,6 +298,9 @@
     float* sk_ws = nullptr; unsigned* sk_flags = nullptr; unsigned sk_epoch = 0;
     float* ks_ws = nullptr; int* ks_cnt = nullptr;
     struct LazyOut { bool active = false; int pitch = 0, rows = 0, shave = 0, conv_index = -1; } lazy;
+    struct FusedJoin { bool armed = false, done = false; const float* skip = nullptr; int pitch = 0, rows = 0, cols = 0; } fuse;
+    unsigned* fj_cnt = nullptr; unsigned fj_count = 0;
+    int arena_fuse_key = 0;
     unsigned* sk_err_host = nullptr; unsigned* sk_err_dev = nullptr;
     bool shared_device = false;
     int precision = 0;
@@ -321,7 +326,7 @@
         for (auto& c : convs) { (void)hipFree(c.wgt); (void)hipFree(c.bias); (void)hipFree(c.wgt16); for (float* p : c.packed) (void)hipFree(p); }
         for (auto& i : ins) { (void)hipFree(i.gamma); (void)hipFree(i.beta); (void)hipFree(i.scale); (void)hipFree(i.shift); (void)hipFree(i.acc); }
         for (void* sp : slabs) (void)hipFree(sp);
-        (void)hipFree(ones); (void)hipFree(zeros); (void)hipFree(sk_ws); (void)hipFree(sk_flags); (void)hipFree(ks_ws); (void)hipFree(ks_cnt); if (sk_err_host) (void)hipHostFree(sk_err_host);
+        (void)hipFree(ones); (void)hipFree(zeros); (void)hipFree(sk_ws); (void)hipFree(sk_flags); (void)hipFree(ks_ws); (void)hipFree(ks_cnt); (void)hipFree(fj_cnt); if (sk_err_host) (void)hipHostFree(sk_err_host);
     }
     int upload_layers(std::vector<Layer>& ls, int& chan_pitch, int& maxc);
     int upload();
@@ -429,6 +434,8 @@
     FAV_HIP(hipMalloc(reinterpret_cast<void**>(&ks_ws), conv3_wino4_ksplit_bytes()));
     FAV_HIP(hipMalloc(reinterpret_cast<void**>(&ks_cnt), 256 * sizeof(int)));
     FAV_HIP(hipMemset(ks_cnt, 0, 256 * sizeof(int)));
+    FAV_HIP(hipMalloc(reinterpret_cast<void**>(&fj_cnt), sizeof(unsigned)));
+    FAV_HIP(hipMemset(fj_cnt, 0, sizeof(unsigned)));
     FAV_HIP(hipHostMalloc(reinterpret_cast<void**>(&sk_err_host), sizeof(unsigned), hipHostMallocMapped));
     *sk_err_host = 0;
     FAV_HIP(hipHostGetDevicePointer(reinterpret_cast<void**>(&sk_err_dev), sk_err_host, 0));
@@ -481,7 +488,7 @@
     prof_pending.push_back(r);
     if ((int)prof_ms.size() <= conv_index) { prof_ms.resize(conv_index + 1, 0.0); prof_macs.resize(conv_index + 1, 0.0); prof_n.resize(conv_index + 1, 0); prof_tile.resize(conv_index + 1, 0); }
     prof_macs[conv_index] = (double)c.OH * c.OW * L.cout * L.cin * L.k * L.k;
-    prof_tile[conv_index] = conv_facts(kernel, c.OH, c.OW, c.COUTp, precision, c.join_skip != nullptr).id;
+    prof_tile[conv_index] = conv_facts(kernel, c.OH, c.OW, c.COUTp, precision, c.join_skip != nullptr || c.fj_skip != nullptr).id;
     return rc;
 }
 
@@ -572,12 +579,23 @@
             const bool want_stats = li + 1 < ls.size() && ls[li + 1].type == L_IN;
             const ConvFacts facts = conv_facts(kernel, c.OH, c.OW, d.coutp, precision, cur.join_skip != nullptr);
             nxt.mblocks = facts.tiles; nxt.ppitch = d.coutp;
-            const bool acc = kernel == CK_WINO4 && want_stats && !pitched_out && cur.join_skip == nullptr &&
-                             (acc_stats_ok(ls, li) || (branch_tail_acc_ok && !top && li + 2 == ls.size() && !tuning().no_acc_stats && precision == 0));
+            const bool tail_acc = branch_tail_acc_ok && !top && li + 2 == ls.size() && !tuning().no_acc_stats && precision == 0;
+            const bool acc = kernel == CK_WINO4 && want_stats && !pitched_out && cur.join_skip == nullptr && (acc_stats_ok(ls, li) || tail_acc);
             if (acc) {
                 DevIN& din = ins[in_cursor];
                 nxt.acc = din.acc + (size_t)acc_parity * stat_acc_words(L.cout); nxt.acc_other = din.acc + (size_t)(acc_parity ^ 1) * stat_acc_words(L.cout);
                 c.stat_acc = nxt.acc;
+                bool one_round = false;
+                const int grid = (tail_acc && fuse.armed && L.cout == 128 && d.coutp == 128 && c.OH == fuse.rows && c.OW == fuse.cols)
+                                     ? conv3_wino4_grid(c.OH, c.OW, L.cout, reserve_cus, ks_ws && ks_cnt, &one_round) : 0;
+                if (one_round) {
+                    c.fj_skip = fuse.skip; c.fj_pitch = fuse.pitch; c.fj_acc_zero = nxt.acc_other;
+                    c.fj_gamma = din.gamma; c.fj_beta = din.beta; c.fj_eps = ls[li + 1].eps;
+                    fj_count += (unsigned)grid;
+                    c.fj_cnt = fj_cnt; c.fj_target = fj_count;
+                    nxt.acc = nullptr; nxt.acc_other = nullptr; nxt.joined = true;
+                    fuse.done = true;
+                }
             }
             if (want_stats && !acc) { rc = alloc((size_t)nxt.mblocks * d.coutp * 2 * sizeof(float), &nxt.partials); if (rc) return rc; }
             if (want_stats && !acc && facts.counts) { float* cp = nullptr; rc = alloc((size_t)nxt.mblocks * sizeof(int), &cp); if (rc) return rc; nxt.counts = reinterpret_cast<int*>(cp); }
@@ -597,6 +615,7 @@
             const int C = (int)L.gamma.size();
             const int M = cur.Hp * cur.Wp;
             if (cur.data == nullptr || C != cur.C) { set_error("network: misplaced InstanceNormalization"); return FAV_EUNSUPPORTED; }
+            if (cur.joined) { cur.joined = false; break; }
             if (cur.acc != nullptr && cur.pre.stages == 0) {
                 cur.pre = Affine();
                 cur.pre.acc1 = cur.acc; cur.pre.acc1_zero = cur.acc_other; cur.pre.gamma1 = d.gamma; cur.pre.beta1 = d.beta; cur.pre.eps1 = L.eps; cur.pre.count1 = M;
@@ -657,9 +676,20 @@
             if (nx < ls.size() && ls[nx].type == L_UP && ls[nx].scale == 2) ++nx;
             const bool join_stats = nx < ls.size() && ls[nx].type == L_IN;
             branch_tail_acc_ok = !lazy_out && !join_stats;
+            fuse = FusedJoin();
+            fuse.armed = branch_tail_acc_ok && !shared_device && !tuning().no_fused_join && skip.pre.stages == 0 && skip.ups == 0;
+            fuse.skip = skip.data + ((size_t)L.shave * skip.P() + L.shave) * skip.C; fuse.pitch = skip.P();
+            fuse.rows = skip.Hp - 2 * L.shave; fuse.cols = skip.Wp - 2 * L.shave;
             rc = run(L.block, br, false, nullptr, nullptr);
-            lazy.active = false; branch_tail_acc_ok = false;
+            const bool fused = fuse.done;
+            lazy.active = false; branch_tail_acc_ok = false; fuse = FusedJoin();
             if (rc) return rc;
+            if (fused) {
+                if (br.pre.stages != 0 || br.ups != 0 || br.C != skip.C) { set_error("internal: a residual join formed by its branch came out pending"); return FAV_EINVAL; }
+                cur = br;
+                cur.partials = nullptr; cur.counts = nullptr;
+                break;
+            }
             if (br.pre.stages != 1 || br.pre.relu1 || br.ups != 0) { set_error("network: residual branch must end in conv + InstanceNormalization"); return FAV_EUNSUPPORTED; }
             if (br.Hp != skip.Hp - 2 * L.shave || br.Wp != skip.Wp - 2 * L.shave || br.C != skip.C) {
                 set_error("network: residual branch output %dx%d does not match the shaved skip %dx%d", br.Wp, br.Hp,
@@ -753,7 +783,9 @@
                   "wrong (two networks running concurrently on one device? see the concurrency note in fav.h)");
         return FAV_EHIP;
     }
-    if (H != curH || W != curW) {
+    const int fuse_key = (!shared_device && !tuning().no_fused_join) ? 1 + reserve_cus : 0;
+    if (H != curH || W != curW || fuse_key != arena_fuse_key) {
+        arena_fuse_key = fuse_key;
         if (!bufs.empty()) {
             FAV_HIP(hipDeviceSynchronize());
             for (void* sp : slabs) (void)hipFree(sp);
@@ -765,6 +797,7 @@
     st = stream; cursor = 0; conv_cursor = 0; in_cursor = 0;
     if (acc_dirty) {
         for (DevIN& i : ins) if (i.acc) FAV_HIP(hipMemsetAsync(i.acc, 0, i.acc_bytes, stream));
+        FAV_HIP(hipMemsetAsync(fj_cnt, 0, sizeof(unsigned), stream)); fj_count = 0;
         acc_dirty = false;
     }
     if (precision == 0 && !tuning().no_acc_stats && !tuning().no_wino) acc_parity ^= 1;
```

Result: no change. 653.7 (-0.6%).
